# antonior92/ip-nonlinear-solver

Hardware: AMD Instinct MI355X
Metric: projected-CG iters/sec (fp64) at n=1e6,m=1e5 (higher is better)
Workload: dtype f64; 1 GPU; config3: sparse banded NLP subproblem, CSR Jacobian bandwidth 15: ONE call ipsolver.qp.projected_cg(H, c, Z, Y, b, trust_radius=1e300, tol=0, max_iter=steps), b a device vector (zeros; x0 = Y(-b) is computed: whether a device vector is zero is not known without reading it) -- priming included; finite trust radius that is never reached (the norm test of qp_subproblem.py:583 formed every iteration, ; n=1000000, m=100000, nnz_A=1500000, nnz_H=2999998, parallelism=single GPU

## Files before the change

include/ipx.h:

```cpp
#ifndef IPX_H
#define IPX_H

#include <stdint.h>

#ifdef __cplusplus
extern "C" {
#endif

#define IPX_OK 0
#define IPX_EINVAL (-1)
#define IPX_ELAUNCH (-2)
#define IPX_ENOTSPD (-3)
#define IPX_ENOMEM (-4)
#define IPX_EUNSUPPORTED (-5)
#define IPX_EILLCOND (-6)

#define IPX_WS_DOUBLES 65536
#define IPX_MAX_PARTIALS 2048

const char *ipx_version(void);
long long ipx_launch_count(void);
long long ipx_read_count(void);
const char *ipx_last_error(void);
int ipx_device_info(int *cu_count, int *lds_bytes, char *arch, int arch_len);
// ... 139 lines not shown
  const int32_t *A_rowptr, *A_colidx; const double *A_val; const int32_t *A_tiles; int64_t A_ntiles;
  const int32_t *At_rowptr, *At_colidx; const double *At_val; const int32_t *At_tiles; int64_t At_ntiles;
  const int32_t *H_rowptr, *H_colidx; const double *H_val; const int32_t *H_tiles; int64_t H_ntiles;
  const double *H_diag;
  void *banded;
  double *x, *p, *r, *Hp;
  double *w, *v, *t;
  const double *lb, *ub;
  double *state;
  double *part1, *part2, *part3, *part4;
  int64_t vec_grid;
  int64_t solver_kind;
  double *pb;
  int64_t H_hmax;
  int64_t H_tile_rows;
  double *r_next;
  const int32_t *A_own;
  int64_t A_span;
  double *fold_ws;
  const int32_t *At_vown;
  int64_t At_qv;
  int64_t A_tile_nnz;
  const uint16_t *At_ell_row;
  const double *At_ell_val;
  const void *H_col16;
  const int32_t *H_rowlen;
  const void *A_col16;
  int64_t no_radius;
  const void *A_off16;
  const int32_t *A_rowfirst;
  int64_t A_rl;
  const int32_t *P_win;
  int64_t P_nspan;
  int64_t P_navn;
  int64_t H_operator;
  int64_t resident;
  void *R_ll;
  int64_t R_hw;
  int64_t *R_seq;
  const double *LR_W;
  const double *LR_state;
  double *LR_part;
  int64_t LR_mem;
  int64_t LR_rows;
  double *xsums;
  int64_t fused_proj;
  const double *A_ell_val;
  const void *A_ell_off16;
  int32_t *r_where;
  int32_t xsums_carry;
  int32_t A_contig;
  double *rguard;
  int32_t radius_guard;
} ipx_cg_args;
#define IPX_CG_MODE_NO_RADIUS 1
#define IPX_CG_MODE_NO_ORTH 2
#define IPX_CG_MODE_CARRIED 4
#define IPX_CG_MODE_GUARD 8
#define IPX_CG_STOP_RADIUS_UNDECIDED 10
#define IPX_CG_STOP_GUARD_LOST 11
double ipx_rguard_start(double sumsq);
double ipx_rguard_step_x(double X, double Q, double alpha);
double ipx_rguard_step_q(double Q, double beta, double gg);
int ipx_cg_guard_resume(const ipx_cg_args *a, int32_t it_stop, void *stream);
int ipx_cg_prime_state_guard(double *state, const double *red, const int32_t *idx7, double tol_in,
                             double radius, double orth_tol, double norm_A, double cancellation,
                             double *rguard, void *stream);
int ipx_cg_resident_ok(const ipx_cg_args *a);
int64_t ipx_cg_resident_ll_words(int32_t nwg, int32_t hw);
void ipx_cg_resident_limits(int32_t *out8);
int32_t ipx_cg_resident_max_global(void);
int ipx_cg_state_size(void);
int ipx_cg_vec_grid(int64_t n);
int ipx_cg_hp(const ipx_cg_args *a, void *stream);
int ipx_cg_iterate(const ipx_cg_args *a, int32_t it_begin, int32_t it_end, void *stream);
int64_t ipx_cg_prime_ws_doubles(const ipx_cg_args *a, int32_t A_ntiles);
int ipx_cg_prime(const ipx_cg_args *a, const int32_t *A_tiles, int32_t A_ntiles, const double *c,
                 const double *b, double *red, double *ws, double tol_in, double radius,
                 double orth_tol, double norm_A, double cancellation, int32_t first_end,
                 int32_t steps, void *stream);
int ipx_cg_prime_state(double *state, const double *red, const int32_t *idx7, double tol_in,
                       double radius, double orth_tol, double norm_A, double cancellation,
                       void *stream);
int ipx_cg_iterate_timed(const ipx_cg_args *a, int32_t it_begin, int32_t it_end,
                         float *ms_out, void *stream);
int ipx_cg_step1(int64_t n, double *state, int32_t it, const double *p1, int32_t np1,
                 const double *x, const double *p, double *r, const double *Hp, const double *lb,
                 const double *ub, double *part2, int32_t grid, void *stream);
int ipx_cg_step2(int64_t n, double *state, int32_t it, int32_t mode, const double *p2,
                 int32_t np2, const double *p3, int32_t np3, const double *p4, int32_t np4,
                 double *x, double *p, const double *g, int32_t grid, void *stream);
typedef struct ipx_pcg_args {
  int64_t m, n;
  const int32_t *A_rowptr, *A_colidx; const double *A_val; const int32_t *A_tiles; int64_t A_ntiles;
  const int32_t *At_rowptr, *At_colidx; const double *At_val; const int32_t *At_tiles; int64_t At_ntiles;
  const double *dinv;
  double *v, *r, *p, *Sp;
  double *t;
  double *state;
  double *part1, *part2;
  int64_t grid;
  const double *binv; const int32_t *border; int64_t nblk;
  double *z, *part3;
  double *rsum; const int32_t *coarse_of, *goff; int64_t ncoarse;
  const double *X; int64_t ldx;
  double *y, *partc;
} ipx_pcg_args;
int ipx_pcg_state_size(void);
int ipx_pcg_iterate(const ipx_pcg_args *a, int32_t it_begin, int32_t it_end, void *stream);
int ipx_pcg_coarse_max(void);
int ipx_pcg_coarse_grid(int64_t ncoarse);
int ipx_pcg_precond_apply(const ipx_pcg_args *a, const double *r, double *z, double *rz,
                          void *stream);
int ipx_csr_aggregate_rows(int64_t ncoarse, const int32_t *A_rowptr, const int32_t *A_colidx,
                           const double *A_val, const int32_t *order, const int32_t *goff,
                           const int32_t *C_rowptr, const int32_t *C_colidx, double *C_val,
                           void *stream);
int ipx_aggregate_greedy(int64_t n, const int32_t *rowptr, const int32_t *colidx, int32_t cap,
                         int32_t *agg);
int ipx_blockjacobi_build(int64_t nblk, const int32_t *rowptr, const int32_t *colidx,
                          const double *val, const int32_t *order, double *binv, int *flag,
                          void *stream);
int ipx_blockjacobi_apply(int64_t m, int64_t nblk, const int32_t *order, const double *binv,
                          const double *r, double *z, double *ws, const double *state,
                          void *stream);
typedef struct ipx_shard2_ext {
  double *s1;
  double *pack;
  int64_t nseg;
  int64_t own_lo[4], own_hi[4];
  int64_t p1_lo[4], p1_hi[4];
  int64_t p3_lo[4], p3_hi[4];
  int64_t p2_lo, p2_hi;
  int64_t p4_lo, p4_hi;
  void *peer;
  int64_t seg_lo[4], seg_hi[4];
  int64_t send_left[4], send_right[4];
  int64_t fuse_comm;
  int64_t res_wg0, res_nwg, res_gwg0, res_gnwg;
} ipx_shard2_ext;
int ipx_cg_shard2_fusable(const ipx_cg_args *a, const ipx_shard2_ext *e);
int ipx_cg_shard2_segment(const ipx_cg_args *a, const ipx_shard2_ext *e, int32_t phase,
                          int32_t it, int32_t mode, void *stream);
int ipx_cg_shard2_iterate(const ipx_cg_args *a, const ipx_shard2_ext *e, int32_t it_begin,
                          int32_t it_end, void *stream);
int ipx_cg_shard2_resident_ok(const ipx_cg_args *a, const ipx_shard2_ext *e);
int ipx_cg_shard2_resident(const ipx_cg_args *a, const ipx_shard2_ext *e, int32_t it_begin,
                           int32_t it_end, void *stream);
int ipx_cg_save_pb(const ipx_cg_args *a, void *stream);

int ipx_peer_handle_bytes(void);
void *ipx_peer_create(int32_t rank, int32_t world, int64_t halo_cap);
int ipx_peer_export(void *peer, void *handle_out);
int ipx_peer_import(void *peer, int32_t rank, const void *handle_in);
int ipx_peer_ready(void *peer);
int64_t ipx_peer_halo_capacity(void *peer);
int ipx_peer_set_timeout(void *peer, double seconds);
int ipx_peer_sequence(void *peer, int64_t *out2);
int64_t ipx_peer_fused_launches(void *peer);
void ipx_peer_destroy(void *peer);
int ipx_peer_allreduce(void *peer, int32_t nq, const double *in, double *out, int *failed,
                       int32_t reps, void *stream);
int ipx_peer_allgather(void *peer, int32_t nq, const double *vals, double *out, int *failed,
                       void *stream);
int ipx_peer_exchange(void *peer, double *v, int32_t nseg, const int64_t *geom, int *failed,
                      void *stream);
// ... 224 lines not shown
```

ip-nonlinear-solver_amd/csrc/banded.hip:

```cpp
#include "ipx_common.h"
#include "pcr_window.h"
#include <vector>

namespace {

constexpr int KMAX = 8;
constexpr int MAX_LEVELS = 8;
constexpr int WIDE_MIN_ROWS = 2048;
constexpr int ITER_TOP_MIN_ROWS = 1024;
constexpr double ITER_ETA_MAX = 0.5;

struct Level {
  int m, k, c, P, q;
  int mR;
  double *band;
  double *Dinv;
  double *L;
  double *V, *W;
  double *rhs;
  double *sol;
};

struct Banded {
  int nlev;
// ... 1167 lines not shown
    }
    if (!partial) return;
  }
  double acc = 0.0;
  for (int r = threadIdx.x; r < T * q; r += blockDim.x) {
    const int64_t g = (int64_t)t0 * q + r;
    if (g < m) {
      const int li = q + r;
      double sum = sB[r] * sx[li];
#pragma unroll
      for (int d = 1; d <= K; ++d) {
        if (g - d >= 0) sum += sB[d * NB + r] * sx[li - d];
        if (g + d < m) sum += sB[d * NB + r + d] * sx[li + d];
      }
      const double res = sw0[r] - sum;
      acc += res * res;
    }
  }
  const double tot = ipx_block_reduce<IPX_SUM>(acc, red_lds);
  if (threadIdx.x == 0) partial[blockIdx.x] = tot;
  IPX_STAMP(7);
}


constexpr int PCR_RMAX = 4 * 66 + 2 * (1 << PCR_LMAX) + 8;
constexpr int PCR_NR = (PCR_RMAX + IPX_BLOCK - 1) / IPX_BLOCK;
constexpr int PCR_TB = 512;

__global__ void __launch_bounds__(IPX_BLOCK)
k_pcr_check(int m, int rows_wg, int nwin, const double *__restrict__ band, int *flags) {
  constexpr int PAD = PCR_PAD;
  constexpr int RS = PCR_RMAX + 2 * PAD;
  __shared__ double pa[2][RS], pr[2][RS];
  const int wg = ipx_xcd_item(blockIdx.x, nwin);
  if (wg < 0) return;
  const int tid = threadIdx.x;
  const PcrWindow win(wg, rows_wg, PCR_LMAX, m, tid);
  const int R = win.R;
  double a[PCR_NR], b[PCR_NR], b0[PCR_NR];
  bool own[PCR_NR];
#pragma unroll
  for (int k = 0; k < PCR_NR; ++k) {
    const int r = tid + k * IPX_BLOCK;
    win.row_load(band, r, a[k], b[k]);
    b0[k] = b[k];
    own[k] = win.own(r);
  }
  pcr_pad_identity<IPX_BLOCK, false>(R, tid, pa, pr);
  const double tiny = 1.3877787807814457e-17;
  for (int s = 0; s < PCR_LMAX; ++s) {
    const int h = 1 << s, cur = s & 1;
#pragma unroll
    for (int k = 0; k < PCR_NR; ++k) {
      const int r = tid + k * IPX_BLOCK;
      if (r < R) { pa[cur][PAD + r] = a[k]; pr[cur][PAD + r] = ipx_rcp_newton(b[k]); }
    }
    ipx_lds_barrier();
    int bits = 0;
#pragma unroll
    for (int k = 0; k < PCR_NR; ++k) {
      const int r = PAD + min(tid + k * IPX_BLOCK, R - 1);
      const double alo = pa[cur][r - h], rlo = pr[cur][r - h];
      const double ahi = pa[cur][r + h], rhi = pr[cur][r + h];
      double none = 0.0;
      pcr_eliminate<false>(a[k], b[k], none, alo, rlo, 0.0, ahi, rhi, 0.0);
      const double bn = b[k];
      if (own[k]) {
        const double aup = (-pa[cur][r + 2 * h] * rhi) * ahi;
        if (!(fmax(fabs(a[k]), fabs(aup)) <= tiny * bn)) bits |= 1;
        if (!(bn > 0.0)) bits |= 2;
        if (!(bn > IPX_PIVOT_RTOL * b0[k])) bits |= 4;
      }
    }
    const bool any0 = __ballot(bits & 1) != 0, any1 = __ballot(bits & 2) != 0;
    const bool any2 = __ballot(bits & 4) != 0;
    if ((tid & (IPX_WAVE - 1)) == 0) {
      if (any0) flags[s + 1] = 1;
      if (any1) flags[PCR_LMAX + 1 + s + 1] = 1;
      if (any2) flags[PCR_LMAX + 1] = 1;
    }
  }
}

template <int QV, int NR, bool ROWS, int TB, bool POST = false>
__global__ void __launch_bounds__(TB)
k_solve_pcr(int m, int rows_wg, int L, int nwin, const double *__restrict__ band,
            const double *__restrict__ w, double *__restrict__ x, double *__restrict__ partial,
            const double *__restrict__ guard, AtvJob atv, RowsJob rows = RowsJob{},
            PostJob post = PostJob{}) {
  constexpr int QA = QV > 0 ? QV : 1;
  constexpr int RS = PCR_RMAX + 2 * PCR_PAD;
  __shared__ double pa[2][RS], pr[2][RS], pd[2][RS];
  __shared__ double sx[PCR_RMAX];
  __shared__ double red_lds[TB / IPX_WAVE];
  constexpr int RWU = ROWS_PRODUCTS / TB;
  const int wg = ipx_xcd_item(blockIdx.x, nwin);
  if (wg < 0) return;
  IPX_STAMP(0);
  int av0 = 0, avn = 0;
  if (QV > 0) {
    av0 = atv.vown[wg];
    avn = atv.vown[wg + 1] - av0;
  }
  const double stop = guard ? *guard : 0.0;
  const int tid = threadIdx.x;
  const PcrWindow win(wg, rows_wg, L, m, tid);
  const int H = win.H, R = win.R;
  const int64_t g0 = win.row(0);
  extern __shared__ double rows_prod[];
  int rcol[ROWS ? RWU : 1];
  double rval[ROWS ? RWU : 1];
  if constexpr (ROWS) {
    const int64_t nnz = (int64_t)m << rows.logL;
    const int64_t e0 = g0 * (1 << rows.logL);
    const int P = R << rows.logL;
#pragma unroll
    for (int u = 0; u < RWU; ++u) {
      const int e = min(tid + u * TB, P - 1);
      const int64_t idx = min(max(e0 + e, (int64_t)0), nnz - 1);
      rcol[u] = rows.col[idx];
      rval[u] = rows.val[idx];
    }
  }
  double a[NR], b[NR], d[NR];
#pragma unroll
  for (int k = 0; k < NR; ++k) {
    const bool in = win.row_load(band, tid + k * TB, a[k], b[k]);
    if constexpr (!ROWS) {
      const double wv = w[win.clamped(tid + k * TB)];
      d[k] = in ? wv : 0.0;
    }
  }
  if constexpr (ROWS) {
    const int Lr = 1 << rows.logL, P = R << rows.logL;
    double xg[RWU];
#pragma unroll
    for (int u = 0; u < RWU; ++u) xg[u] = rows.x[rcol[u]];
#pragma unroll
    for (int u = 0; u < RWU; ++u) {
      const int e = tid + u * TB;
      if (e < P) rows_prod[(e >> rows.logL) * (Lr + 1) + (e & (Lr - 1))] = rval[u] * xg[u];
    }
    ipx_lds_barrier();
#pragma unroll
    for (int k = 0; k < NR; ++k) {
      const int r = tid + k * TB;
      const bool in = win.inside(r);
      double sum = 0.0;
      if (in) {
        const double *pr_ = rows_prod + r * (Lr + 1);
        for (int j = 0; j < Lr; ++j) sum += pr_[j];
      }
      d[k] = in ? 1.0 * sum : 0.0;
    }
  }
  constexpr int QP = (QA + 1) / 2;
  PcrPairTail<QP, TB> tail;
  v2d ar[QP];
  if (QV > 0)
    tail.load(atv.ell_row, atv.ell_val, atv.ell_n, av0, avn, tid, [&](int k, int64_t j) {
      ar[k] = *reinterpret_cast<const v2d *>(atv.r_in + j);
    });
  int pg0 = 0, pgn = 0, pe0 = 0, pen = 0;
  int py0[POST ? POST_PG + 1 : 1], py1[POST ? POST_PG + 1 : 1];
  double pw0[POST ? POST_PG + 1 : 1], pw1[POST ? POST_PG + 1 : 1];
  double pep[POST ? POST_PG : 1], peq[POST ? POST_PG : 1];
  double prc[POST ? POST_PG + 1 : 1], prp[POST ? POST_PG : 1], prq[POST ? POST_PG : 1];
  if constexpr (POST) {
    pg0 = post.own_g[wg]; pgn = post.own_g[wg + 1] - pg0;
    pe0 = post.own_e[wg]; pen = post.own_e[wg + 1] - pe0;
    const ipx_group_tab &T = post.T;
#pragma unroll
    for (int k = 0; k < POST_PG; ++k) {
      const int i = pg0 + min(tid + k * TB, max(pgn - 1, 0));
      const int gi = min(i, max(post.ng - 1, 0));
      const int c = T.c0 + gi;
      py0[k] = post.yrow[gi]; py1[k] = post.yrow[post.nitems + gi];
      pw0[k] = post.yval[gi]; pw1[k] = post.yval[post.nitems + gi];
      pep[k] = T.grp2[2 * gi]; peq[k] = T.grp2[2 * gi + 1];
      prc[k] = post.r[c]; prp[k] = post.r[c + T.dp]; prq[k] = post.r[c + T.dq];
    }
    {
      const int e = min(pe0 + min(tid, max(pen - 1, 0)), max(post.nitems - post.ng - 1, 0));
      const int i = post.ng + e;
      py0[POST_PG] = post.yrow[min(i, post.nitems - 1)];
      py1[POST_PG] = post.yrow[post.nitems + min(i, post.nitems - 1)];
      pw0[POST_PG] = post.yval[min(i, post.nitems - 1)];
      pw1[POST_PG] = post.yval[post.nitems + min(i, post.nitems - 1)];
      prc[POST_PG] = post.r[T.gen0 + e];
    }
  }
  if (stop != 0.0) return;
  IPX_STAMP(1);
  double a0[NR], b0[NR], w0[NR];
#pragma unroll
  for (int k = 0; k < NR; ++k) { a0[k] = a[k]; b0[k] = b[k]; w0[k] = d[k]; }
  IPX_STAMP(2);
  pcr_pad_identity<TB, true>(R, tid, pa, pr, pd);
  pcr_levels<NR, TB>(L, R, tid, a, b, d, pa, pr, pd);
  IPX_STAMP(3);
  pcr_solution_to_lds<NR, TB>(win, tid, d, b, sx, x);
  if (!partial && QV == 0 && !POST) return;
  ipx_lds_barrier();
  IPX_STAMP(6);
  if (QV > 0) {
    const double gacc = tail.apply(
        sx, H, atv.sign, tid, atv.g_out,
        [&](int k, int64_t, int half) { return half ? ar[k].y : ar[k].x; }, [](int, bool, bool) {});
    pcr_partial_pair<TB>(gacc, red_lds, atv.part3, wg, nwin, tid);
    if (!partial) return;
  }
  if constexpr (POST) {
    const ipx_group_tab &T = post.T;
    const int wlim = R - 1;
    double acc = 0.0;
#pragma unroll
    for (int k = 0; k < POST_PG; ++k) {
      if (tid + k * TB < pgn) {
        const int gi = pg0 + tid + k * TB;
        const int c = T.c0 + gi, cp = c + T.dp, cq = c + T.dq;
        const double u0 = sx[min(max((int)(py0[k] - g0), 0), wlim)];
        const double u1 = sx[min(max((int)(py1[k] - g0), 0), wlim)];
        double sum = 0.0;
        sum += pw0[k] * u0;
        sum += pw1[k] * u1;
        const double yj = 1.0 * sum;
        const double ap = copysign(1.0, pep[k]), sp = fabs(pep[k]);
        const double aq = copysign(1.0, peq[k]), sq = fabs(peq[k]);
        const double rc = prc[k], rp = prp[k], rq = prq[k];
        double i11, i12, i22, wgt;
        ipx_group_inverse(true, ap, sp, aq, sq, i11, i12, i22, wgt);
        const double wp = cp > c ? ap * rc + sp * rp : sp * rp + ap * rc;
        const double wq = cq > c ? aq * rc + sq * rq : sq * rq + aq * rc;
        const double ep = ap * yj, eq = aq * yj;
        const double tp = i11 * wp + i12 * wq;
        const double tq = i12 * wp + i22 * wq;
        const double vp = tp - (i11 * ep + i12 * eq);
        const double vq = tq - (i12 * ep + i22 * eq);
        double s3 = yj + ap * vp;
        s3 += aq * vq;
        double gc = -1.0 * s3;
        gc += 1.0 * rc;
        double gp = -1.0 * (sp * vp);
        gp += 1.0 * rp;
        double gq = -1.0 * (sq * vq);
        gq += 1.0 * rq;
        post.g[c] = gc; post.g[cp] = gp; post.g[cq] = gq;
        acc += gc * gc;
        acc += gp * gp;
        acc += gq * gq;
      }
    }
    if (tid < pen) {
      const int e = pe0 + tid;
      const double u0 = sx[min(max((int)(py0[POST_PG] - g0), 0), wlim)];
      const double u1 = sx[min(max((int)(py1[POST_PG] - g0), 0), wlim)];
      double sum = 0.0;
      sum += pw0[POST_PG] * u0;
      sum += pw1[POST_PG] * u1;
      double gc = -1.0 * (1.0 * sum);
      gc += 1.0 * prc[POST_PG];
      post.g[T.gen0 + e] = gc;
      acc += gc * gc;
    }
    const double gtot = ipx_block_reduce<IPX_SUM>(acc, red_lds);
    if (tid == 0) {
      post.part[wg] = gtot;
      post.part[post.count + wg] = 0.0;
      for (int k = wg + nwin; k < post.count; k += nwin) {
        post.part[k] = 0.0;
        post.part[post.count + k] = 0.0;
      }
    }
    if (!partial) return;
  }
  const double acc = pcr_own_residual<NR, TB>(win, tid, a0, b0, w0, pa[0], sx);
  const double tot = ipx_block_reduce<IPX_SUM>(acc, red_lds);
  if (tid == 0) partial[wg] = tot;
  IPX_STAMP(7);
}

template <int QV>
int launch_solve_pcr_q(const LevDev &lv, int L, const double *w, double *x, double *partial,
                       int *npartial, const double *guard, const AtvJob &atv, hipStream_t st) {
  const int rows_wg = DEC_CHUNKS * lv.q;
  const int grid = (lv.P + DEC_CHUNKS - 1) / DEC_CHUNKS;
  if (npartial) *npartial = grid;
  constexpr int NRL = (PCR_RMAX + PCR_TB - 1) / PCR_TB;
  if (rows_wg + 2 * (1 << L) <= PCR_TB)
    hipLaunchKernelGGL((k_solve_pcr<QV, 1, false, PCR_TB>), dim3(ipx_xcd_grid(grid)), dim3(PCR_TB),
                       0, st, lv.m, rows_wg, L, grid, lv.band, w, x, partial, guard, atv, RowsJob{});
  else
    hipLaunchKernelGGL((k_solve_pcr<QV, NRL, false, PCR_TB>), dim3(ipx_xcd_grid(grid)),
                       dim3(PCR_TB), 0, st, lv.m, rows_wg, L, grid, lv.band, w, x, partial, guard,
                       atv, RowsJob{});
  IPX_CHECK_LAUNCH();
  return IPX_OK;
}

int launch_solve_pcr_rows(const LevDev &lv, int L, const RowsJob &rows, double *x,
                          double *partial, int *npartial, const double *guard, hipStream_t st,
                          const PostJob *post = nullptr) {
  const int rows_wg = DEC_CHUNKS * lv.q;
  const int R = rows_wg + 2 * (1 << L);
  if (R > PCR_TB || ((int64_t)R << rows.logL) > (int64_t)ROWS_PRODUCTS)
    return IPX_EUNSUPPORTED;
  const int grid = (lv.P + DEC_CHUNKS - 1) / DEC_CHUNKS;
  if (npartial) *npartial = grid;
  const size_t lds = (size_t)R * ((1 << rows.logL) + 1) * sizeof(double);
  constexpr int dyn = (int)(LDS_LIMIT - 44 * 1024);
  if (post) {
    allow_dynamic_lds<k_solve_pcr<0, 1, true, PCR_TB, true>>(dyn);
    hipLaunchKernelGGL((k_solve_pcr<0, 1, true, PCR_TB, true>), dim3(ipx_xcd_grid(grid)),
                       dim3(PCR_TB), lds, st, lv.m, rows_wg, L, grid, lv.band, nullptr, x, partial,
                       guard, AtvJob{}, rows, *post);
  } else {
    allow_dynamic_lds<k_solve_pcr<0, 1, true, PCR_TB>>(dyn);
    hipLaunchKernelGGL((k_solve_pcr<0, 1, true, PCR_TB>), dim3(ipx_xcd_grid(grid)), dim3(PCR_TB),
                       lds, st, lv.m, rows_wg, L, grid, lv.band, nullptr, x, partial, guard,
                       AtvJob{}, rows);
  }
  IPX_CHECK_LAUNCH();
  return IPX_OK;
}

int pcr_tail_per_lane(int qv) { return (qv * (DOWN_T - IPX_WAVE) + 1 + PCR_TB - 1) / PCR_TB; }

int launch_solve_pcr(const LevDev &lv, int L, const double *w, double *x, double *partial,
                     int *npartial, const double *guard, hipStream_t st,
                     const AtvJob *atv = nullptr, int qv = 0) {
  const AtvJob none{};
  if (!atv || qv <= 0)
    return launch_solve_pcr_q<0>(lv, L, w, x, partial, npartial, guard, none, st);
  const int per = pcr_tail_per_lane(qv);
  if (per <= 2) return launch_solve_pcr_q<2>(lv, L, w, x, partial, npartial, guard, *atv, st);
  if (per <= 4) return launch_solve_pcr_q<4>(lv, L, w, x, partial, npartial, guard, *atv, st);
  if (per <= 6) return launch_solve_pcr_q<6>(lv, L, w, x, partial, npartial, guard, *atv, st);
  if (per <= 8) return launch_solve_pcr_q<8>(lv, L, w, x, partial, npartial, guard, *atv, st);
  return IPX_EINVAL;
}

template <int QV, int XN, bool PRIME = false, bool CONTIG = false>
__global__ void __launch_bounds__(PCR_TB)
k_step1_solve_tail(int m, int rows_wg, int L, int nwin, const double *__restrict__ band,
                   ipx_fused_proj_job J) {
  constexpr int TB = PCR_TB;
  constexpr int PAD = 1 << PCR_LMAX;
  constexpr int RS = PCR_RMAX + 2 * PAD;
  constexpr int QSP = IPX_FP_SPAN / TB;
  constexpr int RLA = IPX_FP_ROW;
  constexpr int FW = IPX_BLOCK, FU = 6;
  constexpr int QP = (QV + 1) / 2;
  __shared__ double pa[2][RS], pr[2][RS], pd[2][RS];
  __shared__ double sx[PCR_RMAX];
  __shared__ double span[IPX_FP_SPAN];
  __shared__ double red_lds[TB / IPX_WAVE];
  __shared__ double fold_lds[FW / IPX_WAVE];
  const int tid = threadIdx.x, wg = ipx_xcd_item(blockIdx.x, nwin);
  if (wg < 0) return;
  const int av0 = J.vown[wg], avn = J.vown[wg + 1] - av0;
  const int c_lo = J.win[2 * wg], nspan = J.win[2 * wg + 1] - c_lo;
  static_assert(!PRIME || XN == 1, "the priming's projection forms no radius test");
  double stop, rtg = 0.0, tol = 0.0;
  if constexpr (PRIME) {
    stop = J.guard ? *J.guard : 0.0;
  } else {
    stop = J.st[ST_STOP];
    rtg = J.st[J.parity ? ST_RTG1 : ST_RTG0];
    tol = J.st[ST_TOL];
  }
  double rgX = 0.0, rgQ = 0.0;
  if constexpr (XN == 3) {
    if (wg == 0 && tid == 0) { rgX = J.xs_comp[IPX_RG_X]; rgQ = J.xs_comp[IPX_RG_Q]; }
  }
  double ft[FU];
  if (!PRIME && tid < FW) {
#pragma unroll
    for (int u = 0; u < FU; ++u) {
      const int i = tid + u * FW;
      const double ld = J.p1[max(min(i, J.np1 - 1), 0)];
      ft[u] = i < J.np1 ? ld : 0.0;
    }
// ... 907 lines not shown
  }
  if (h->decoupled && w != x && h->pcr_L > 0 && h->lev[0].k == 1)
    return launch_solve_pcr(to_dev(h->lev[0], nullptr), h->pcr_L, w, x, partial, npartial, guard,
                            st);
  if (h->chunk_pending) {
    const int rc = ensure_chunks(h, st);
    if (rc != IPX_OK) return rc;
    return fast_solve(h, w, x, partial, npartial, guard, st);
  }
  if (h->decoupled && w != x)
    return solve_decoupled_k(to_dev(h->lev[0], nullptr), w, x, h->rinv, partial, npartial, guard,
                             st);
  if (h->iter_N > 0 && !h->decoupled) {
    if (w == x && partial) return IPX_EINVAL;
    return iter_solve(h, w, x, partial, npartial, guard, st);
  }
  if (h->wide) return IPX_EUNSUPPORTED;
  int rc = fast_down0(h, w, h->ybuf, guard, st);
  if (rc != IPX_OK) return rc;
  if (!decoupled_scalar(h)) {
    if (!h->upper_done) {
      rc = factor_upper(h, st);
      if (rc != IPX_OK) return rc;
    }
    rc = fast_middle(h, guard, st);
    if (rc != IPX_OK) return rc;
  }
  switch (h->lev[0].k) {
#define CO(kk) case kk: return launch_correct_oop<kk>(h, x, w, partial, npartial, guard, st)
    CO(1); CO(2); CO(3); CO(4); CO(5); CO(6); CO(7); CO(8);
#undef CO
  }
  return IPX_EINVAL;
}
}

int ipx_banded_resid_count(void *handle) {
  if (!handle) return 0;
  Banded *h = (Banded *)handle;
  const Level &l0 = h->lev[0];
  if (h->fast && h->nlev > 1 && h->decoupled)
    return (l0.P + DEC_CHUNKS - 1) / DEC_CHUNKS;
  if (h->fast && h->nlev > 1 && h->iter_N == 0) return (l0.m + IPX_BLOCK - 1) / IPX_BLOCK;
  const int grid = (l0.m + IPX_BLOCK - 1) / IPX_BLOCK;
  return grid > 256 ? 256 : grid;
}

extern "C" int ipx_banded_decoupled_geometry(void *handle, int32_t *out) {
  if (!handle || !out) return 0;
  Banded *h = (Banded *)handle;
  const Level &l0 = h->lev[0];
  if (!(h->fast && h->nlev > 1 && h->decoupled))
    return 0;
  out[0] = DEC_CHUNKS * l0.q;
  out[1] = (l0.P + DEC_CHUNKS - 1) / DEC_CHUNKS;
  return 1;
}

int ipx_banded_solve_resid_atv_launch(void *handle, const double *w, double *x, double *partial,
                                      int *npartial, const int32_t *At_rowptr,
                                      const int32_t *At_colidx, const double *At_val,
                                      const double *r_in, double *g_out, const int32_t *vown,
                                      int qv, double *part3, const double *guard,
                                      hipStream_t st, const uint16_t *ell_row,
                                      const double *ell_val, int64_t ell_n, double sign) {
  if (!handle || !w || !x || !partial || w == x || (sign != 1.0 && sign != -1.0)) return IPX_EINVAL;
  int32_t geo[2];
  if (!ipx_banded_decoupled_geometry(handle, geo)) return IPX_EINVAL;
  Banded *h = (Banded *)handle;
  const AtvJob job{At_rowptr, At_colidx, At_val, r_in, g_out, vown, part3, ell_row, ell_val, ell_n,
                   sign};
  if (h->pcr_L > 0 && ell_row && ell_val)
    return launch_solve_pcr(to_dev(h->lev[0], nullptr), h->pcr_L, w, x, partial, npartial, guard,
                            st, &job, qv);
  if (h->chunk_pending) {
    const int rc = ensure_chunks(h, st);
    if (rc != IPX_OK) return rc;
    if (!ipx_banded_decoupled_geometry(handle, geo)) return IPX_EINVAL;
  }
  return solve_decoupled_k(to_dev(h->lev[0], nullptr), w, x, h->rinv, partial, npartial, guard, st,
                           &job, qv);
}

int ipx_banded_fused_proj_ok(void *handle, int rl, int64_t nspan, int qv) {
  int32_t geo[2];
  if (!handle || !ipx_banded_decoupled_geometry(handle, geo)) return IPX_EUNSUPPORTED;
  Banded *h = (Banded *)handle;
  if (h->pcr_L <= 0 || h->lev[0].k != 1 || geo[0] + 2 * (1 << h->pcr_L) > PCR_TB)
    return IPX_EUNSUPPORTED;
  if (rl < 1 || rl > IPX_FP_ROW || nspan < 1 || nspan > IPX_FP_SPAN || qv < 1 ||
      pcr_tail_per_lane(qv) > 6)
    return IPX_EUNSUPPORTED;
  return IPX_OK;
}

int ipx_banded_fused_proj_launch(void *handle, const ipx_fused_proj_job &job, int *npartial,
                                 hipStream_t st) {
  if (job.prime ? (job.xn != 1 || (job.sign != 1.0 && job.sign != -1.0))
                : (!job.st || !job.p1 || !job.Hp || !job.where))
    return IPX_EINVAL;
  if (!job.r_in || !job.g_out || job.g_out == job.r_in ||
      !job.A_ell_val || !job.A_ell_off16 || !job.A_rowfirst || !job.win || !job.vown ||
      !job.ell_row || !job.ell_val || !job.v || !job.part3 || !job.part4 ||
      (job.n & 1) || (job.xn == 0 && (!job.x || !job.p || !job.part2)) ||
      (job.xn == 2 && (!job.xs_raw || !job.xs_comp || job.nraw < 1)) ||
      (job.xn == 3 && !job.xs_comp) || job.xn < 0 || job.xn > 3)
    return IPX_EINVAL;
  if (ipx_banded_fused_proj_ok(handle, job.rl, 1, job.qv) != IPX_OK) return IPX_EUNSUPPORTED;
  Banded *h = (Banded *)handle;
  const LevDev lv = to_dev(h->lev[0], nullptr);
  const int grid = (lv.P + DEC_CHUNKS - 1) / DEC_CHUNKS;
  if (job.xn == 2 && job.ncomp > grid) return IPX_EINVAL;
  if (npartial) *npartial = grid;
  const int per = pcr_tail_per_lane(job.qv);
  if (per <= 2) return launch_step1_solve_tail_q<2>(lv, h->pcr_L, job, grid, st);
  if (per <= 4) return launch_step1_solve_tail_q<4>(lv, h->pcr_L, job, grid, st);
  return launch_step1_solve_tail_q<6>(lv, h->pcr_L, job, grid, st);
}

int ipx_banded_pcr_view(void *handle, ipx_pcr_view *out) {
  if (!handle || !out) return 0;
  int32_t g2[2];
  if (!ipx_banded_decoupled_geometry(handle, g2)) return 0;
  Banded *h = (Banded *)handle;
  if (h->pcr_L <= 0) return 0;
  out->m = h->lev[0].m;
  out->rows_wg = g2[0];
  out->nwg = g2[1];
  out->L = h->pcr_L;
  out->band = h->lev[0].band;
  return 1;
}

int ipx_banded_solve_resid_launch(void *handle, const double *w, double *x, double *partial,
                                  int *npartial, const double *guard, hipStream_t st) {
  if (!handle || !w || !x || !partial || w == x) return IPX_EINVAL;
  Banded *h = (Banded *)handle;
  if (h->fast) return fast_solve(h, w, x, partial, npartial, guard, st);
  int rc = ipx_banded_solve_guarded(handle, w, x, guard, st);
  if (rc != IPX_OK) return rc;
  return ipx_banded_residual_launch(handle, w, x, partial, npartial, guard, st);
}

int ipx_banded_solve_rows_launch(void *handle, const int32_t *col, const double *val,
                                 const double *xin, int logL, double *x, double *partial,
                                 int *npartial, const double *guard, hipStream_t st,
                                 const ipx_post_job *pj) {
  if (!handle || !col || !val || !xin || !x || !partial || logL < 0 || logL > 4) return IPX_EINVAL;
  Banded *h = (Banded *)handle;
  if (!(h->fast && h->nlev > 1 && h->decoupled && h->pcr_L > 0)) return IPX_EUNSUPPORTED;
  const LevDev lv = to_dev(h->lev[0], nullptr);
  if (lv.k != 1) return IPX_EUNSUPPORTED;
  if (!pj)
    return launch_solve_pcr_rows(lv, h->pcr_L, RowsJob{col, val, xin, logL}, x, partial, npartial,
                                 guard, st);
  if (pj->rows_wg != DEC_CHUNKS * lv.q || pj->reach > 1 || (1 << h->pcr_L) < pj->reach)
    return IPX_EUNSUPPORTED;
  if ((lv.P + DEC_CHUNKS - 1) / DEC_CHUNKS > pj->count) return IPX_EUNSUPPORTED;
  PostJob post{pj->own_g, pj->own_e, pj->ng, pj->nitems, pj->T, pj->yrow, pj->yval, pj->r, pj->g,
               pj->part, pj->count};
  return launch_solve_pcr_rows(lv, h->pcr_L, RowsJob{col, val, xin, logL}, x, partial, npartial,
                               guard, st, &post);
}

int ipx_banded_solve_guarded(void *handle, const double *w, double *x, const double *guard,
                             hipStream_t st) {
// ... 85 lines not shown
```

ip-nonlinear-solver_amd/csrc/cg.hip:

```cpp
#include "ipx_common.h"
#include <algorithm>
#include <vector>


namespace {

IPX_STAMP_DECL(ipx_dbg_cg);
#define CG_STAMP(k) IPX_STAMP_TO(ipx_dbg_cg, k)

constexpr int VB = IPX_BLOCK;

constexpr int VU = 8;

typedef ipx_own_ranges OwnRanges;
struct ipx_no_peer {};
template <bool PEER> struct peer_arg { typedef ipx_no_peer type; };
template <> struct peer_arg<true> { typedef ipx_peer_job type; };
static OwnRanges own_all(int64_t n) {
  OwnRanges o;
  for (int k = 0; k < 4; ++k) { o.lo[k] = 0; o.hi[k] = 0; }
  o.hi[0] = n;
  return o;
}

// ... 770 lines not shown
  }
  int rpv[(IPX_SPMV_TILE_ROWS / IPX_BLOCK) + 1];
#pragma unroll
  for (int q = 0; q <= IPX_SPMV_TILE_ROWS / IPX_BLOCK; ++q)
    rpv[q] = rowptr[r0 + min(tid + q * IPX_BLOCK, nrows)] - s;
  CG_STAMP(11);
  ipx_lds_barrier();
  CG_STAMP(12);
#pragma unroll
  for (int u = 0; u < U; ++u) {
    const int jj = s + tid + u * IPX_BLOCK;
    if (jj < e) prod[jj - s] = v[u] * span[c[u]];
  }
#pragma unroll
  for (int q = 0; q <= IPX_SPMV_TILE_ROWS / IPX_BLOCK; ++q) {
    const int i = tid + q * IPX_BLOCK;
    if (i <= nrows) rp[i] = rpv[q];
  }
  ipx_lds_barrier();
  double yq[IPX_SPMV_TILE_ROWS / IPX_BLOCK];
#pragma unroll
  for (int q = 0; q < IPX_SPMV_TILE_ROWS / IPX_BLOCK; ++q) {
    const int i = tid + q * IPX_BLOCK;
    yq[q] = 0.0;
    if (i < nrows) {
      const int a = rp[i], b = rp[i + 1];
      double sum = 0.0;
      for (int k = a; k < b; ++k) sum += prod[k];
      yq[q] = 1.0 * sum;
    }
  }
  CG_STAMP(13);
  if (!NOXN2) {
    const double tot = ipx_block_reduce<IPX_SUM>(sx, lds);
    if (tid == 0) { part2[tile] = tot; part2[ntiles + tile] = 0.0; }
  }
#pragma unroll
  for (int q = 0; q < IPX_SPMV_TILE_ROWS / IPX_BLOCK; ++q) {
    const int i = tid + q * IPX_BLOCK;
    if (i < nrows) w[r0 + i] = yq[q];
  }
  CG_STAMP(14);
}

struct CompactJob {
  const double *in[3];
  double *out[3];
  int count[3], halves[3], G[3], first[4];
};
__global__ void __launch_bounds__(IPX_BLOCK)
k_compact_partials(CompactJob job, const double *__restrict__ guard) {
  __shared__ double lds[IPX_BLOCK / IPX_WAVE];
  if (guard && *guard != 0.0) return;
  int k = 0;
  while (k < 2 && (int)blockIdx.x >= job.first[k + 1]) ++k;
  const int b = blockIdx.x - job.first[k];
  const int half = b / job.G[k], chunk = b - half * job.G[k];
  const int lo = chunk * 1024, len = min(1024, job.count[k] - lo);
  const double v = ipx_sum_partials<IPX_SUM>(job.in[k] + (int64_t)half * job.count[k] + lo, len, lds);
  if (threadIdx.x == 0) job.out[k][half * job.G[k] + chunk] = v;
}

__global__ void __launch_bounds__(IPX_BLOCK)
k_cg_save_pb(const double *__restrict__ p, const int32_t *__restrict__ tiles, int ntiles,
             int hmax, double *__restrict__ pb, double *__restrict__ xs_tag) {
  const int idx = blockIdx.x * blockDim.x + threadIdx.x;
  if (idx == 0 && xs_tag) *xs_tag = 0.0;
  if (idx >= ntiles * 2 * hmax) return;
  const int t = idx / (2 * hmax), j = idx - t * 2 * hmax;
  const int r0 = tiles[t], r1 = tiles[t + 1];
  const double v = j < hmax ? p[r0 + j] : p[r1 - hmax + (j - hmax)];
  pb[idx] = v;
  pb[(int64_t)ntiles * 2 * hmax + idx] = v;
}

__global__ void __launch_bounds__(VB)
k_cg_settle_r(int64_t n, const int32_t *__restrict__ where, const double *__restrict__ src,
              double *__restrict__ dst) {
  if (*where == 0) return;
  for (int64_t i = (int64_t)blockIdx.x * VB + threadIdx.x; i < n; i += (int64_t)gridDim.x * VB)
    dst[i] = src[i];
}

__global__ void k_xsums_void(double *xs_tag) { *xs_tag = 0.0; }

__global__ void k_rguard_advance(const double *__restrict__ st, int parity, double *rg) {
  if (st[ST_STOP] != 0.0) return;
  const double gg = st[parity ? ST_RTG0 : ST_RTG1];
  rg[IPX_RG_Q] = ipx_rguard::step_q(rg[IPX_RG_Q], st[ST_BETA], gg);
  rg[IPX_RG_X] = rg[IPX_RG_T];
}

__global__ void __launch_bounds__(IPX_BLOCK)
k_rguard_sums(int64_t n, const double *__restrict__ x, const double *__restrict__ p,
              double *__restrict__ comp) {
  __shared__ double lds[3 * (IPX_BLOCK / IPX_WAVE)];
  const int64_t per = (n + XS_STRIDE - 1) / XS_STRIDE;
  const int64_t lo = min((int64_t)blockIdx.x * per, n), hi = min(lo + per, n);
  double acc[3] = {0.0, 0.0, 0.0}, out[3];
  for (int64_t i = lo + threadIdx.x; i < hi; i += IPX_BLOCK) {
    const double xv = x[i], pv = p[i];
    acc[0] += xv * xv;
    acc[1] += xv * pv;
    acc[2] += pv * pv;
  }
  ipx_block_sum_multi<3>(acc, lds, out);
  if (threadIdx.x == 0) {
#pragma unroll
    for (int q = 0; q < 3; ++q) comp[q * XS_STRIDE + blockIdx.x] = out[q];
  }
}

struct RangeJob {
  const double *ptr[4][4];
  int count[4][4];
  int npieces;
  int active;
};

__global__ void __launch_bounds__(256)
k_cg_range_pack(RangeJob job, double *__restrict__ out, const double *__restrict__ guard) {
  __shared__ double lds[4 * 4];
  if (guard && *guard != 0.0) return;
  double acc[4] = {0.0, 0.0, 0.0, 0.0};
  for (int pc = 0; pc < job.npieces; ++pc) {
    double red[4];
    ipx_sum_partials_multi<4>(job.ptr[pc], job.count[pc], lds, red);
#pragma unroll
    for (int q = 0; q < 4; ++q) acc[q] += red[q];
  }
  if (threadIdx.x < 4 && ((job.active >> threadIdx.x) & 1)) out[threadIdx.x] = acc[threadIdx.x];
}

struct HaloPlan {
  int nseg;
  int seg_lo[4], own_lo[4], own_hi[4], seg_hi[4], send_left[4], send_right[4];
};

__global__ void __launch_bounds__(256)
k_cg_pack_comm(RangeJob job, double *__restrict__ out, ipx_peer_view pv, uint32_t seq,
               HaloPlan hp, double *__restrict__ g, uint32_t hseq, double *__restrict__ st) {
  __shared__ double lds[4 * 4];
  __shared__ double vals[IPX_MAX_PEERS * 4];
  const int tid = threadIdx.x;
  if (st[ST_STOP] == 7.0) return;
  const long long deadline = (long long)wall_clock64() + pv.timeout_ticks;
  if (blockIdx.x == 0) {
    double acc[4] = {0.0, 0.0, 0.0, 0.0};
    for (int pc = 0; pc < job.npieces; ++pc) {
      double red[4];
      ipx_sum_partials_multi<4>(job.ptr[pc], job.count[pc], lds, red);
#pragma unroll
      for (int q = 0; q < 4; ++q) acc[q] += red[q];
    }
    const int slot = seq & (IPX_PEER_SLOTS - 1);
    if (tid < 4 * pv.world) {
      const int r = tid >> 2, q = tid & 3;
      if ((job.active >> q) & 1) {
        const double mine = q == 0 ? acc[0] : (q == 1 ? acc[1] : (q == 2 ? acc[2] : acc[3]));
        ipx_ll_store(pv.mbox[r] + ipx_peer_scal_word(slot, pv.rank, q), mine, seq);
      }
    }
    bool ok = true;
    if (tid < 4 * pv.world) {
      const int r = tid >> 2, q = tid & 3;
      double v = 0.0;
// ... 190 lines not shown
               : step2_hp_forms<PEER, false, 4, 5>(box, c16, xsum, guard);
}


template <bool PEER>
int launch_step1_box(const ipx_cg_args *a, int it, const double *p1, int np1, int np2,
                     const OwnRanges &own, typename peer_arg<PEER>::type pj, hipStream_t st) {
  const ipx_boxschur_args *b = (const ipx_boxschur_args *)a->banded;
  const ipx_group_tab T = ipx_boxschur_tab(b);
  hipLaunchKernelGGL(step1_box_kernel<PEER>(ipx_group_mode(T)), dim3(ipx_xcd_grid(np2)),
                     dim3(IPX_BLOCK), 0, st, a->state, it & 1, p1, np1, a->x, a->p, a->r, a->Hp,
                     a->lb, a->ub, a->part2, np2, (int)b->ng, (int)b->ngen, T, b->gen_cols,
                     (int)b->ny, b->up, own, step1_box_rounds(b), pj);
  IPX_CHECK_LAUNCH();
  return IPX_OK;
}

template <bool PEER>
int launch_step1_ar(const ipx_cg_args *a, const LoopPlan &P, int it, const double *p1, int np1,
                    bool no_xn2, bool carried, bool guard, typename peer_arg<PEER>::type pj,
                    hipStream_t st) {
  if (carried && (PEER || no_xn2 || !a->xsums)) return IPX_EINVAL;
  if (guard && (PEER || no_xn2 || carried || !a->rguard)) return IPX_EINVAL;
  if (a->A_tile_nnz != 0) return IPX_EINVAL;
  const int qs = (int)((a->A_span + IPX_BLOCK - 1) / IPX_BLOCK);
  const auto k = step1_ar_kernel<PEER>(qs, guard ? 3 : carried ? 2 : no_xn2 ? 1 : 0,
                                       a->A_col16 != nullptr);
  if (!k) return IPX_EINVAL;
  const int nraw = carried ? (int)a->H_ntiles : 0;
  hipLaunchKernelGGL(k, dim3(ipx_xcd_grid((int)a->A_ntiles)), dim3(IPX_BLOCK), 0, st, (int)a->n,
                     a->state, it & 1, p1, np1, a->x, a->p, a->r, a->r_next, a->Hp, a->A_rowptr,
                     a->A_colidx, a->A_val, a->A_tiles, (int)a->A_ntiles, a->A_own, a->w,
                     a->part2, (const uint16_t *)a->A_col16, pj, carried ? a->xsums : nullptr,
                     nraw, guard ? a->rguard : carried ? a->xsums + 3 * nraw + 1 : nullptr,
                     carried ? P.xs_ncomp : 0, it);
  IPX_CHECK_LAUNCH();
  return IPX_OK;
}

template <bool PEER>
int launch_step2_hp(const ipx_cg_args *a, int it, int mode, const double *p2, int np2,
                    const double *p3, int np3, const double *p4, int np4,
                    typename peer_arg<PEER>::type pj, const ipx_xsums_job &xs, hipStream_t st,
                    const double *g = nullptr) {
  const bool guard = (mode & 8) != 0;
  const bool xsum = !guard && xs.raw != nullptr && (xs.write != 0 || (mode & 4) != 0);
  if ((mode & 4) && (!xsum || !xs.in || PEER || a->lb)) return IPX_EINVAL;
  if (guard && (!xs.raw || !xs.in || xs.write || (mode & 4) || PEER || a->lb)) return IPX_EINVAL;
  const bool small = a->H_tile_rows > 0 && a->H_tile_rows + 2 * a->H_hmax <= 3 * IPX_BLOCK;
  const bool c16 = a->H_col16 != nullptr && a->H_rowlen != nullptr;
  const auto k = step2_hp_kernel<PEER>(a->H_diag != nullptr, small, a->lb != nullptr, c16, xsum,
                                       guard);
  if (!k) return IPX_EINVAL;
  const int64_t half = a->H_ntiles * 2 * a->H_hmax;
  const double *pb_in = a->pb + (it & 1) * half;
  double *pb_out = a->pb + ((it + 1) & 1) * half;
  double *g_halo = PEER ? a->r : nullptr;
  hipLaunchKernelGGL(k, dim3(ipx_xcd_grid((int)a->H_ntiles)), dim3(IPX_BLOCK), 0, st, (int)a->n,
                     a->state, it & 1, mode, p2, np2, p3, np3, p4, np4, a->x, a->p,
                     g ? g : (const double *)a->r, a->H_rowptr, a->H_colidx, a->H_val, a->H_tiles,
                     (int)a->H_ntiles, a->H_diag, a->Hp, a->part1, (int)a->H_hmax, pb_in, pb_out,
                     (const uint16_t *)a->H_col16, a->H_rowlen, pj, g_halo, xs);
  IPX_CHECK_LAUNCH();
  return IPX_OK;
}

double *xsums_tag(const ipx_cg_args *a) {
  return a->xsums ? a->xsums + 3 * a->H_ntiles : nullptr;
}

int launch_save_pb(const ipx_cg_args *a, hipStream_t st) {
  const int tot = (int)(a->H_ntiles * 2 * a->H_hmax);
  hipLaunchKernelGGL(k_cg_save_pb, dim3((tot + IPX_BLOCK - 1) / IPX_BLOCK), dim3(IPX_BLOCK), 0, st,
                     a->p, a->H_tiles, (int)a->H_ntiles, (int)a->H_hmax, a->pb, xsums_tag(a));
  IPX_CHECK_LAUNCH();
  return IPX_OK;
}

int launch_lowrank(const ipx_cg_args *a, bool has_base, const double *guard, hipStream_t st) {
  return ipx_lowrank_cg_launch(a->n, a->LR_rows, (int)a->LR_mem, a->LR_W, a->LR_state, a->LR_part,
                               a->p, a->Hp, a->H_diag, has_base ? 1 : 0, a->part1, guard, st);
}

int launch_hp(const ipx_cg_args *a, const LoopPlan &P, const double *guard, hipStream_t st) {
  int rc = IPX_OK;
  switch (P.hp) {
    case HP_OPERATOR:
      return IPX_OK;
    case HP_LOWRANK:
      return launch_lowrank(a, false, guard, st);
    case HP_DENSE: {
      int np = 0;
      rc = ipx_dense_gemv_launch((int)a->n, (int)a->n, a->H_val, a->n, a->p, 1.0, a->H_diag, 0.0,
                                 nullptr, a->Hp, a->part1, &np, guard, st);
      break;
    }
    case HP_CSR: {
      ipx_csr_view H{(int)a->n, (int)a->n, a->H_rowptr, a->H_colidx, a->H_val, a->H_tiles,
                     (int)a->H_ntiles};
      rc = ipx_spmv_launch(H, a->p, 1.0, a->H_diag, 0.0, nullptr, a->Hp, a->part1, guard, st);
      break;
    }
  }
  if (!rc && P.lowrank_tail) rc = launch_lowrank(a, true, guard, st);
  if (rc || P.hp != HP_CSR || !P.fused_hp) return rc;
  return launch_save_pb(a, st);
}

struct Compactor {
  const ipx_cg_args *a;
  CompactJob job;
  const double *guard;
  int n = 0, used = 0;
  Compactor(const ipx_cg_args *args, const double *g) : a(args), guard(g) { job.first[0] = 0; }
  bool add(const double *&ptr, int &count, int halves, int limit) {
    if (!a->fold_ws || count <= limit || n >= 3) return false;
    const int G = (count + 1023) / 1024;
    if (used + halves * G > IPX_FOLD_WS_DOUBLES) return false;
    job.in[n] = ptr; job.count[n] = count; job.halves[n] = halves; job.G[n] = G;
    job.out[n] = a->fold_ws + used;
    job.first[n + 1] = job.first[n] + halves * G;
    ptr = a->fold_ws + used;
    count = G;
    used += halves * G;
    ++n;
    return true;
  }
  int launch(hipStream_t st) {
    if (n == 0) return IPX_OK;
    for (int k = n; k < 3; ++k) job.first[k + 1] = job.first[n];
    hipLaunchKernelGGL(k_compact_partials, dim3(job.first[n]), dim3(IPX_BLOCK), 0, st, job, guard);
    IPX_CHECK_LAUNCH();
    n = 0;
    job.first[0] = 0;
    return IPX_OK;
  }
};


struct HalfArgs {
  int it;
  int mode;
  const double *guard;
  const OwnRanges *own = nullptr;
  const ipx_peer_job *peer = nullptr;
  Compactor *cmp = nullptr;
  ipx_xsums_job xs{nullptr, nullptr, it, 0};
  hipEvent_t *ev = nullptr;
  bool flip = false, first = true;
  const double *g = nullptr;
};
#define MARK(i) do { if (h.ev) (void)hipEventRecord(h.ev[i], st); } while (0)

int launch_projection_half(const ipx_cg_args *a, const LoopPlan &P, const HalfArgs &h,
                           const double *p1, int np1, int *np2, int *np3, int *np4,
                           hipStream_t st) {
  MARK(0);
  int rc;
  if (h.cmp) {
    h.cmp->add(p1, np1, 2, 2048);
    rc = h.cmp->launch(st);
    if (rc) return rc;
  }
  if (P.proj == PJ_STEP1_SOLVE_TAIL) {
    if (h.peer || h.own) return IPX_EINVAL;
    const bool carried = (h.mode & 4) != 0, guarded = (h.mode & 8) != 0;
    if (carried && ((h.mode & 1) || !a->xsums)) return IPX_EINVAL;
    if (guarded && ((h.mode & 5) || !a->rguard)) return IPX_EINVAL;
    const int nraw = carried ? (int)a->H_ntiles : 0;
    ipx_fused_proj_job J{};
    J.st = a->state; J.parity = h.it & 1; J.p1 = p1 + np1; J.np1 = np1;
    J.r_in = h.flip ? a->r_next : a->r; J.Hp = a->Hp; J.g_out = h.flip ? a->r : a->r_next;
    J.xn = guarded ? 3 : carried ? 2 : (h.mode & 1) ? 1 : 0;
    J.x = a->x; J.p = a->p; J.part2 = a->part2;
    J.xs_raw = carried ? a->xsums : nullptr; J.nraw = nraw;
    J.xs_comp = guarded ? a->rguard : carried ? a->xsums + 3 * nraw + 1 : nullptr;
    J.ncomp = carried ? P.xs_ncomp : 0; J.it = h.it;
    J.A_ell_val = a->A_ell_val; J.A_ell_off16 = (const uint16_t *)a->A_ell_off16;
    J.contig = a->A_contig != 0;
    J.A_rowfirst = a->A_rowfirst; J.rl = (int)a->A_rl; J.win = a->P_win; J.n = a->n;
    J.vown = a->At_vown; J.qv = (int)a->At_qv; J.ell_row = a->At_ell_row; J.ell_val = a->At_ell_val;
    J.v = a->v; J.part3 = a->part3; J.part4 = a->part4;
    J.where = a->r_where; J.first = h.first ? 1 : 0; J.dest = h.flip ? 0 : 1;
    MARK(1); MARK(2);
    int np = 0;
    rc = ipx_banded_fused_proj_launch(a->banded, J, &np, st);
    if (rc) return rc;
    *np2 = *np3 = *np4 = np;
// ... 57 lines not shown
        rc = ipx_banded_solve_resid_atv_launch(a->banded, a->w, a->v, a->part4, np4, a->At_rowptr,
                                               a->At_colidx, a->At_val, r_in, a->r, a->At_vown,
                                               (int)a->At_qv, a->part3, h.guard, st,
                                               a->At_ell_row, a->At_ell_val, a->n);
        if (rc) return rc;
        *np3 = *np4;
        MARK(3);
        MARK(4);
      } else {
        if (a->solver_kind == 1)
          rc = ipx_boxschur_solve((const ipx_boxschur_args *)a->banded, a->w, a->v, a->part4, np4,
                                  h.guard, st);
        else
          rc = ipx_banded_solve_resid_launch(a->banded, a->w, a->v, a->part4, np4, h.guard, st);
        if (rc) return rc;
        MARK(3);
        ipx_csr_view At{(int)a->n, (int)a->m, a->At_rowptr, a->At_colidx, a->At_val, a->At_tiles,
                        (int)a->At_ntiles};
        rc = ipx_spmv_launch(At, a->v, -1.0, nullptr, 1.0, r_in, a->r, a->part3, h.guard, st);
        if (rc) return rc;
        MARK(4);
      }
      MARK(5);
      break;
    }
    case PJ_STEP1_SOLVE_TAIL:
      return IPX_EINVAL;
    case PJ_DENSE: {
      const int n = (int)a->n, m = (int)a->m, M = ((m + 31) / 32) * 32;
      int np = 0;
      rc = ipx_dense_gemv_launch(m, n, a->A_val, n, a->r, 1.0, nullptr, 0.0, nullptr, a->w,
                                 nullptr, &np, h.guard, st);
      if (rc) return rc;
      rc = ipx_dense_gemv_launch(M, M, (const double *)a->banded, M, a->w, 1.0, nullptr, 0.0,
                                 nullptr, a->v, nullptr, &np, h.guard, st);
      if (rc) return rc;
      rc = ipx_dense_gemv_launch(n, m, a->At_val, m, a->v, -1.0, nullptr, 1.0, a->r, a->r,
                                 a->part3, np3, h.guard, st);
      if (rc) return rc;
      rc = ipx_dense_gemv_launch(m, n, a->A_val, n, a->r, 1.0, nullptr, 0.0, nullptr, a->t,
                                 a->part4, np4, h.guard, st);
      if (rc) return rc;
      break;
    }
  }
  return IPX_OK;
}

int launch_update_half(const ipx_cg_args *a, const LoopPlan &P, const HalfArgs &h,
                       const double *p2, int np2, const double *p3, int np3, const double *p4,
                       int np4, hipStream_t st) {
  int rc;
  if (h.cmp) {
    if (!(h.mode & 13)) h.cmp->add(p2, np2, 2, 1024);
    h.cmp->add(p3, np3, 2, 2048);
    if (!(h.mode & 2)) h.cmp->add(p4, np4, 1, 1024);
    rc = h.cmp->launch(st);
    if (rc) return rc;
  }
  const double *g = h.g ? h.g : a->r;
  if (P.step2 == S2_FUSED_HP) {
    MARK(6);
    rc = h.peer ? launch_step2_hp<true>(a, h.it, h.mode, p2, np2, p3, np3, p4, np4, *h.peer, h.xs,
                                        st)
                : launch_step2_hp<false>(a, h.it, h.mode, p2, np2, p3, np3, p4, np4,
                                         ipx_no_peer{}, h.xs, st, g);
    if (!rc && P.lowrank_tail) rc = launch_lowrank(a, true, h.guard, st);
  } else {
    if (h.peer) return IPX_EINVAL;
    hipLaunchKernelGGL(k_cg_step2, dim3(ipx_xcd_grid((int)a->vec_grid)), dim3(VB), 0, st, a->n,
                       a->state, h.it & 1, h.mode, p2, np2, p3, np3, p4, np4, a->x, a->p, g,
                       (int)a->vec_grid);
    IPX_CHECK_LAUNCH();
    MARK(6);
    rc = launch_hp(a, P, h.guard, st);
  }
  if (rc) return rc;
  MARK(7);
  return IPX_OK;
}
#undef MARK

int cg_iterate(const ipx_cg_args *a, const LoopPlan &P, int32_t it_begin, int32_t it_end,
               hipStream_t st, hipEvent_t *ev) {
  if (P.proj == PJ_DENSE) {
    if (ev) return IPX_EINVAL;
  } else if (!ev && it_end > it_begin && ipx_cg_resident_ok(a)) {
    int rc = ipx_cg_resident_launch(a, it_begin, it_end, P.np1, P.np2, P.np3, P.np4, st);
    if (rc || !P.fused_hp) return rc;
    return launch_save_pb(a, st);
  }
  const double *guard = a->state + ST_STOP;
  if (a->xsums && !P.xsums && it_end > it_begin) {
    hipLaunchKernelGGL(k_xsums_void, dim3(1), dim3(1), 0, st, xsums_tag(a));
    IPX_CHECK_LAUNCH();
  }
  for (int it = it_begin; it < it_end; ++it) {
    const bool carried = P.xsums && !P.guard && (it > it_begin || a->xsums_carry != 0);
    Compactor cmp(a, guard);
    HalfArgs h{it, (P.proj == PJ_NONE ? 2 : 0) | (P.no_xn2 ? 1 : 0) | (carried ? 4 : 0) |
                       (P.guard ? 8 : 0), guard};
    if (P.proj != PJ_DENSE) h.cmp = &cmp;
    h.xs = ipx_xsums_job{a->xsums,
                         P.guard ? a->rguard : carried ? a->xsums + 3 * a->H_ntiles + 1 : nullptr,
                         it, P.xsums && !P.guard ? 1 : 0};
    h.ev = ev;
    h.first = it == it_begin;
    h.flip = P.proj == PJ_STEP1_SOLVE_TAIL && ((it - it_begin) & 1) != 0;
    if (P.proj == PJ_STEP1_SOLVE_TAIL) h.g = h.flip ? a->r : a->r_next;
    int np2 = 0, np3 = 0, np4 = 0;
    int rc = launch_projection_half(a, P, h, a->part1, P.np1, &np2, &np3, &np4, st);
    if (rc) return rc;
    rc = launch_update_half(a, P, h, a->part2, np2, a->part3, np3, a->part4, np4, st);
    if (rc) return rc;
  }
  if (P.proj == PJ_STEP1_SOLVE_TAIL && it_end > it_begin) {
    hipLaunchKernelGGL(k_cg_settle_r, dim3(ipx_grid_for(a->n, VB * 4, 1024)), dim3(VB), 0, st, a->n,
                       a->r_where, (const double *)a->r_next, a->r);
    IPX_CHECK_LAUNCH();
  }
  return IPX_OK;
}
}

IPX_STAMP_EXPORT(ipx_debug_stamps_cg, ipx_dbg_cg)

extern "C" {

int ipx_cg_state_size(void) { return ST_SIZE; }
int ipx_cg_vec_grid(int64_t n) { return ipx_grid_for(n, VB * 2, 512); }

int ipx_cg_step1(int64_t n, double *state, int32_t it, const double *p1, int32_t np1,
                 const double *x, const double *p, double *r, const double *Hp, const double *lb,
                 const double *ub, double *part2, int32_t grid, void *stream) {
  if (n < 0 || !state || !p1 || !part2 || grid < 1) return IPX_EINVAL;
  hipLaunchKernelGGL(k_cg_step1, dim3(ipx_xcd_grid(grid)), dim3(VB), 0, (hipStream_t)stream, n,
                     state, it & 1, p1, np1, x, p, r, Hp, lb, ub, part2, grid, own_all(n));
  IPX_CHECK_LAUNCH();
  return IPX_OK;
}

int ipx_cg_step2(int64_t n, double *state, int32_t it, int32_t mode, const double *p2,
                 int32_t np2, const double *p3, int32_t np3, const double *p4, int32_t np4,
                 double *x, double *p, const double *g, int32_t grid, void *stream) {
  if (n < 0 || !state || grid < 1) return IPX_EINVAL;
  hipLaunchKernelGGL(k_cg_step2, dim3(ipx_xcd_grid(grid)), dim3(VB), 0, (hipStream_t)stream, n,
                     state, it & 1, mode, p2, np2, p3, np3, p4, np4, x, p, g, grid);
  IPX_CHECK_LAUNCH();
  return IPX_OK;
}

static OwnRanges own_of(const ipx_shard2_ext *e) {
  OwnRanges o;
  for (int k = 0; k < 4; ++k) {
    o.lo[k] = k < e->nseg ? e->own_lo[k] : 0;
    o.hi[k] = k < e->nseg ? e->own_hi[k] : 0;
  }
  return o;
}

static int launch_pack(const ipx_cg_args *a, const ipx_shard2_ext *e, const RangeJob &job,
                       double *out, bool with_halo, hipStream_t st) {
  ipx_peer *peer = (ipx_peer *)e->peer;
  if (!peer) {
    hipLaunchKernelGGL(k_cg_range_pack, dim3(1), dim3(256), 0, st, job, out,
                       (const double *)nullptr);
    IPX_CHECK_LAUNCH();
    return IPX_OK;
  }
  if (peer->view.world > IPX_MAX_PEERS || !ipx_peer_ready(peer)) return IPX_EINVAL;
  HaloPlan hp;
  hp.nseg = 0;
  int64_t moved = 0;
  if (with_halo && peer->view.world > 1) {
    hp.nseg = (int)e->nseg;
    int64_t inl = 0, inr = 0, outl = 0, outr = 0;
    for (int k = 0; k < hp.nseg; ++k) {
      hp.seg_lo[k] = (int)e->seg_lo[k]; hp.seg_hi[k] = (int)e->seg_hi[k];
      hp.own_lo[k] = (int)e->own_lo[k]; hp.own_hi[k] = (int)e->own_hi[k];
      hp.send_left[k] = (int)e->send_left[k]; hp.send_right[k] = (int)e->send_right[k];
      if (hp.seg_lo[k] > hp.own_lo[k] || hp.own_hi[k] > hp.seg_hi[k] || hp.send_left[k] < 0 ||
          hp.send_right[k] < 0 || hp.send_left[k] + hp.send_right[k] > 2 * (hp.own_hi[k] - hp.own_lo[k]))
        return IPX_EINVAL;
      inl += hp.own_lo[k] - hp.seg_lo[k]; inr += hp.seg_hi[k] - hp.own_hi[k];
      outl += hp.send_left[k]; outr += hp.send_right[k];
    }
    if (inl > peer->view.cap || inr > peer->view.cap || outl > peer->view.cap || outr > peer->view.cap)
      return IPX_EINVAL;
    moved = inl + inr + outl + outr;
    if (++peer->hseq == 0) ++peer->hseq;
  }
  if (++peer->seq == 0) ++peer->seq;
  const int halo_wg = hp.nseg ? (int)std::min<int64_t>(16, std::max<int64_t>(1, (moved + 511) / 512)) : 0;
  hipLaunchKernelGGL(k_cg_pack_comm, dim3(1 + halo_wg), dim3(256), 0, st, job, out, peer->view,
                     peer->seq, hp, a->r, peer->hseq, a->state);
  IPX_CHECK_LAUNCH();
  return IPX_OK;
// ... 192 lines not shown
    const double nx2 = q[1 + 3 * pj], nz2 = q[2 + 3 * pj], naz2 = q[3 + 3 * pj];
    const double nz = sqrt(nz2), naz = sqrt(naz2);
    const double orth = (nz == 0.0 || norm_A == 0.0) ? 0.0 : naz / (norm_A * nz);
    const bool stepped = taken && taken[pj] != 0.0;
    if (orth > orth_tol || (!stepped && nz2 < canc2 * nx2)) bad = true;
    if (!stepped && nx2 > 0.0) margin = fmin(margin, nz2 / nx2);
  }
  const double rt_g = q[5];
  const double tr_distance = radius - sqrt(q[0]);
  if (!(tr_distance >= 1e-25)) bad = true;
  double tol = tol_in;
  if (tol_in != tol_in) tol = fmax(fmin(0.01 * sqrt(rt_g), 0.1 * rt_g), 1e-25);
  for (int k = 0; k < ST_SIZE; ++k) st[k] = 0.0;
  st[ST_RTG0] = rt_g;
  st[ST_TOL] = tol;
  st[ST_RADIUS] = radius;
  st[ST_ORTH_RHS] = orth_tol * norm_A;
  st[ST_MARGIN] = margin;
  st[ST_PRIME_STEPS] = taken ? taken[0] + taken[1] : 0.0;
  st[ST_STOP] = bad ? 9.0 : 0.0;
  if (rguard) {
    rguard[IPX_RG_X] = ipx_rguard::start(q[0]);
    rguard[IPX_RG_Q] = ipx_rguard::start(rt_g);
    rguard[IPX_RG_T] = 0.0;
  }
}

__global__ void k_cg_prime_state(double *st, const double *__restrict__ red, ipx_prime_idx ix,
                                 double tol_in, double radius, double orth_tol, double norm_A,
                                 double canc2, double *rguard) {
  if (threadIdx.x != 0 || blockIdx.x != 0) return;
  prime_state_body(st, red, ix, tol_in, radius, orth_tol, norm_A, canc2, nullptr, rguard);
}

struct PrimeFolds {
  const double *part[6];
  int count[6], slot[6], n;
  int single[6];
};
#define PR_SKIP 14
#define PR_TAKEN 16
struct PrimeStep {
  const double *cz, *ct;
  int ncz, nct, base, pj;
  int pairs;
};
__device__ void prime_fold4(const double *pz, int npz, const double *pt, int npt, int pairs,
                            double *lds, double (&out)[4]) {
  const double *parts[4] = {pz, pairs ? pz + npz : pz, pt, pairs ? pt + npt : pt};
  const int counts[4] = {npz, pairs ? npz : 0, npt, pairs ? npt : 0};
  ipx_sum_partials_multi<4>(parts, counts, lds, out);
}
__device__ void prime_fold_step(double *red, const PrimeStep &c, double *lds) {
  if (red[PR_SKIP + c.pj] != 0.0) return;
  double out[4];
  prime_fold4(c.cz, c.ncz, c.ct, c.nct, c.pairs, lds, out);
  if (threadIdx.x == 0) {
    red[c.base] = out[0]; red[c.base + 1] = out[1];
    red[c.base + 2] = out[2]; red[c.base + 3] = out[3];
    red[PR_TAKEN + c.pj] = 1.0;
  }
  __syncthreads();
}
__global__ void __launch_bounds__(IPX_BLOCK)
k_prime_decide(double *red, const double *pz, int npz, const double *pt, int npt, int pairs,
               int base, int xslot, int pj, double orth_tol, double norm_A, double canc2,
               const double *__restrict__ norm_A2_dev, PrimeStep prev, int have_prev) {
  __shared__ double lds[4 * (IPX_BLOCK / IPX_WAVE)];
  if (have_prev) prime_fold_step(red, prev, lds);
  if (norm_A2_dev) norm_A = sqrt(*norm_A2_dev);
  double out[4];
  prime_fold4(pz, npz, pt, npt, pairs, lds, out);
  if (threadIdx.x != 0) return;
  red[base] = out[0]; red[base + 1] = out[1];
  red[base + 2] = out[2]; red[base + 3] = out[3];
  const double nx2 = red[xslot], nz2 = out[0], naz2 = out[2];
  const double nz = sqrt(nz2), naz = sqrt(naz2);
  const double orth = (nz == 0.0 || norm_A == 0.0) ? 0.0 : naz / (norm_A * nz);
  const bool need = orth > orth_tol || nz2 < canc2 * nx2;
  red[PR_SKIP + pj] = need ? 0.0 : 1.0;
  red[PR_TAKEN + pj] = 0.0;
}

__global__ void __launch_bounds__(IPX_BLOCK)
k_cg_prime_state_folds(double *st, double *red, PrimeFolds f, ipx_prime_idx ix, double tol_in,
                       double radius, double orth_tol, double norm_A, double canc2,
                       const double *__restrict__ radius_dev,
                       const double *__restrict__ norm_A2_dev, PrimeStep last, int have_last,
                       double *rguard) {
  if (radius_dev) radius = *radius_dev;
  if (norm_A2_dev) norm_A = sqrt(*norm_A2_dev);
  __shared__ double lds[12 * (IPX_BLOCK / IPX_WAVE)];
  const double *parts[12];
  int counts[12];
#pragma unroll
  for (int j = 0; j < 6; ++j) {
    const bool on = j < f.n, two = on && !f.single[j];
    parts[2 * j] = on ? f.part[j] : f.part[0];
    parts[2 * j + 1] = two ? f.part[j] + f.count[j] : f.part[0];
    counts[2 * j] = on ? f.count[j] : 0;
    counts[2 * j + 1] = two ? f.count[j] : 0;
  }
  double out[12];
  if (f.n > 0) {
    ipx_sum_partials_multi<12>(parts, counts, lds, out);
    if (threadIdx.x == 0) {
#pragma unroll
      for (int j = 0; j < 6; ++j)
        if (j < f.n) { red[f.slot[j]] = out[2 * j]; red[f.slot[j] + 1] = out[2 * j + 1]; }
    }
    __syncthreads();
  }
  if (have_last) prime_fold_step(red, last, lds);
  if (threadIdx.x == 0)
    prime_state_body(st, red, ix, tol_in, radius, orth_tol, norm_A, canc2,
                     have_last ? red + PR_TAKEN : nullptr, rguard);
}

int ipx_cg_prime_state_guard(double *state, const double *red, const int32_t *idx7,
                             double tol_in, double radius, double orth_tol, double norm_A,
                             double cancellation, double *rguard, void *stream) {
  if (!state || !red || !idx7) return IPX_EINVAL;
  ipx_prime_idx ix;
  for (int k = 0; k < 7; ++k) ix.i[k] = idx7[k];
  hipLaunchKernelGGL(k_cg_prime_state, dim3(1), dim3(64), 0, (hipStream_t)stream, state, red, ix,
                     tol_in, radius, orth_tol, norm_A, cancellation * cancellation, rguard);
  IPX_CHECK_LAUNCH();
  return IPX_OK;
}

int ipx_cg_prime_state(double *state, const double *red, const int32_t *idx7, double tol_in,
                       double radius, double orth_tol, double norm_A, double cancellation,
                       void *stream) {
  return ipx_cg_prime_state_guard(state, red, idx7, tol_in, radius, orth_tol, norm_A, cancellation,
                                  nullptr, stream);
}

static int prime_solve(const ipx_cg_args *a, const double *w, double *v, void *stream) {
  if (a->solver_kind == 1)
    return ipx_boxschur_solve((const ipx_boxschur_args *)a->banded, w, v, nullptr, nullptr, nullptr,
                              stream);
  return ipx_banded_solve(a->banded, w, v, stream);
}
struct PrimeRed {
  double *red, *ws;
  int64_t off;
  PrimeFolds f;
  int spmv(const ipx_csr_view &M, const double *x, double alpha, const double *diag, double beta,
           const double *yin, double *yout, int slot, hipStream_t st) {
    double *part = ws + off;
    off += 2 * (int64_t)M.ntiles;
    f.part[f.n] = part; f.count[f.n] = M.ntiles; f.slot[f.n] = slot; f.single[f.n] = 0; ++f.n;
    return ipx_spmv_launch(M, x, alpha, diag, beta, yin, yout, part, nullptr, st);
  }
  void single(const double *part, int count, int slot) {
    f.part[f.n] = part; f.count[f.n] = count; f.slot[f.n] = slot; f.single[f.n] = 1; ++f.n;
  }
};

static int prime_project(const ipx_cg_args *a, const ipx_csr_view &A, const ipx_csr_view &At,
                         const double *x, double *z, PrimeRed &R, int base, bool have_xnorm,
                         double sign, hipStream_t st) {
  int rc = have_xnorm ? IPX_OK : ipx_norms(a->n, x, R.red + base + 4, R.ws + R.off, st);
  if (rc) return rc;
  rc = ipx_spmv_launch(A, x, 1.0, nullptr, 0.0, nullptr, a->w, nullptr, nullptr, st);
  if (rc) return rc;
  rc = prime_solve(a, a->w, a->v, st);
  if (rc) return rc;
  rc = R.spmv(At, a->v, -sign, nullptr, sign, x, z, base, st);
  if (rc) return rc;
  return R.spmv(A, z, 1.0, nullptr, 0.0, nullptr, a->t, base + 2, st);
}
// ... 24 lines not shown
                             int base, bool have_xnorm, double sign, hipStream_t st) {
  if (P.proj != PJ_SOLVE_TAIL && P.proj != PJ_STEP1_SOLVE_TAIL)
    return prime_project(a, A, At, x, z, R, base, have_xnorm, sign, st);
  int rc = have_xnorm ? IPX_OK : ipx_norms(a->n, x, R.red + base + 4, R.ws + R.off, st);
  if (rc) return rc;
  const int cap = (int)((a->m + 255) / 256) + 8;
  double *pz = R.ws + R.off, *pt = pz + 2 * cap;
  R.off += 3 * (int64_t)cap;
  int np = 0;
  rc = prime_project_tail(a, P, A, x, z, pz, pt, &np, sign, nullptr, st);
  if (rc) return rc;
  R.single(pz, np, base);
  R.single(pt, np, base + 2);
  return IPX_OK;
}

static int prime_project_stepped(const ipx_cg_args *a, const LoopPlan &P,
                                 const ipx_csr_view &A, const ipx_csr_view &At, const double *x, double *z, PrimeRed &R,
                                 int base, int xslot, int pj, bool have_xnorm, double sign,
                                 double orth_tol, double norm_A, const double *norm_A2_dev,
                                 double canc2, const PrimeStep *prev, PrimeStep *step,
                                 hipStream_t st) {
  const int n0 = R.f.n;
  int rc;
  const double *skip = R.red + PR_SKIP + pj;
  if (P.proj == PJ_SOLVE_TAIL || P.proj == PJ_STEP1_SOLVE_TAIL) {
    if (!have_xnorm) {
      rc = ipx_norms(a->n, x, R.red + base + 4, R.ws + R.off, st);
      if (rc) return rc;
    }
    const int cap = (int)((a->m + 255) / 256) + 8;
    double *pz = R.ws + R.off, *pt = pz + 2 * cap, *cz = pt + cap, *ct = cz + 2 * cap;
    R.off += 6 * (int64_t)cap;
    int np = 0, npc = 0;
    rc = prime_project_tail(a, P, A, x, z, pz, pt, &np, sign, nullptr, st);
    if (rc) return rc;
    hipLaunchKernelGGL(k_prime_decide, dim3(1), dim3(IPX_BLOCK), 0, st, R.red, pz, np, pt, np, 0,
                       base, xslot, pj, orth_tol, norm_A, canc2, norm_A2_dev,
                       prev ? *prev : PrimeStep{}, prev ? 1 : 0);
    IPX_CHECK_LAUNCH();
    rc = prime_project_tail(a, P, A, z, z, cz, ct, &npc, 1.0, skip, st);
    if (rc) return rc;
    *step = PrimeStep{cz, ct, npc, npc, base, pj, 0};
    return IPX_OK;
  }
  rc = prime_project(a, A, At, x, z, R, base, have_xnorm, sign, st);
  if (rc) return rc;
  const double *pz = R.f.part[n0], *pt = R.f.part[n0 + 1];
  const int npz = R.f.count[n0], npt = R.f.count[n0 + 1];
  R.f.n = n0;
  hipLaunchKernelGGL(k_prime_decide, dim3(1), dim3(IPX_BLOCK), 0, st, R.red, pz, npz, pt, npt, 1,
                     base, xslot, pj, orth_tol, norm_A, canc2, norm_A2_dev,
                     prev ? *prev : PrimeStep{}, prev ? 1 : 0);
  IPX_CHECK_LAUNCH();
  if (a->solver_kind == 1)
    rc = ipx_boxschur_solve((const ipx_boxschur_args *)a->banded, a->t, a->v, nullptr, nullptr, skip,
                            st);
  else
    rc = ipx_banded_solve_guarded(a->banded, a->t, a->v, skip, st);
  if (rc) return rc;
  double *cz = R.ws + R.off;
  R.off += 2 * (int64_t)At.ntiles;
  double *ct = R.ws + R.off;
  R.off += 2 * (int64_t)A.ntiles;
  rc = ipx_spmv_launch(At, a->v, -1.0, nullptr, 1.0, z, z, cz, skip, st);
  if (rc) return rc;
  rc = ipx_spmv_launch(A, z, 1.0, nullptr, 0.0, nullptr, a->t, ct, skip, st);
  if (rc) return rc;
  *step = PrimeStep{cz, ct, At.ntiles, A.ntiles, base, pj, 1};
  return IPX_OK;
}

int64_t ipx_cg_prime_ws_doubles(const ipx_cg_args *a, int32_t A_ntiles) {
  if (!a) return -1;
  return 2 * (5 * a->At_ntiles + 4 * (int64_t)A_ntiles + a->H_ntiles) + 4096;
}

int ipx_cg_prime(const ipx_cg_args *a, const int32_t *A_tiles, int32_t A_ntiles, const double *c,
                 const double *b, double *red, double *ws, double tol_in, double radius,
                 double orth_tol, double norm_A, double cancellation, int32_t first_end,
                 int32_t steps, void *stream) {
  return ipx_cg_prime_dev(a, A_tiles, A_ntiles, c, b, red, ws, tol_in, radius, nullptr, orth_tol,
                          norm_A, nullptr, cancellation, first_end, steps, nullptr, 0, 0,
                          (hipStream_t)stream);
}

}

int ipx_cg_prime_dev(const ipx_cg_args *a, const int32_t *A_tiles, int32_t A_ntiles,
                     const double *c, const double *b, double *red, double *ws, double tol_in,
                     double radius, const double *radius_dev, double orth_tol, double norm_A,
                     const double *norm_A2_dev, double cancellation, int32_t first_end,
                     int steps, const double *c_part, int32_t c_npart, int x_is_zero,
                     hipStream_t stream) {
  if (!a || !c || !red || !ws || !A_tiles || a->solver_kind > 1 || a->m <= 0 || a->H_operator ||
      !a->H_rowptr || !a->t || first_end < 0 || a->LR_W)
    return IPX_EINVAL;
  hipStream_t st = (hipStream_t)stream;
  const LoopPlan P = plan_of(a);
  const ipx_csr_view A{(int)a->m, (int)a->n, a->A_rowptr, a->A_colidx, a->A_val, A_tiles, A_ntiles};
  const ipx_csr_view At{(int)a->n, (int)a->m, a->At_rowptr, a->At_colidx, a->At_val, a->At_tiles,
                        (int)a->At_ntiles};
  const ipx_csr_view Hm{(int)a->n, (int)a->n, a->H_rowptr, a->H_colidx, a->H_val, a->H_tiles,
                        (int)a->H_ntiles};
  if (ipx_cg_prime_ws_doubles(a, A_ntiles) > IPX_WS_DOUBLES) return IPX_EUNSUPPORTED;
  PrimeRed R{red, ws, 0, PrimeFolds{}};
  int rc;
  const double *t = c;
  if (b) {
    rc = prime_solve(a, b, a->v, stream);
    if (rc) return rc;
    rc = R.spmv(At, a->v, -1.0, nullptr, 0.0, nullptr, a->x, 12, st);
    if (rc) return rc;
    rc = R.spmv(Hm, a->x, 1.0, a->H_diag, 1.0, c, a->Hp, 4, st);
    if (rc) return rc;
    t = a->Hp;
  } else if (!x_is_zero &&
             hipMemsetAsync(a->x, 0, (size_t)a->n * sizeof(double), st) != hipSuccess) {
    return IPX_ELAUNCH;
  }
  const double canc2 = cancellation * cancellation;
  PrimeStep s1{}, s2{};
  if (b || !steps) {
    const bool c_known = !b && c_part && c_npart > 0;
    if (c_known) {
      PrimeFolds &f = R.f;
      f.part[f.n] = c_part; f.count[f.n] = c_npart; f.slot[f.n] = 4; f.single[f.n] = 0; ++f.n;
    }
    rc = prime_project_any(a, P, A, At, t, a->r, R, 0, b != nullptr || c_known, 1.0, st);
    if (rc) return rc;
    rc = prime_project_any(a, P, A, At, a->r, a->p, R, 6, true, -1.0, st);
    if (rc) return rc;
  } else {
    rc = prime_project_stepped(a, P, A, At, t, a->r, R, 0, 4, 0, false, 1.0, orth_tol, norm_A,
                               norm_A2_dev, canc2, nullptr, &s1, st);
    if (rc) return rc;
    rc = prime_project_stepped(a, P, A, At, a->r, a->p, R, 6, 0, 1, true, -1.0, orth_tol, norm_A,
                               norm_A2_dev, canc2, &s1, &s2, st);
    if (rc) return rc;
  }
  const int32_t idx_b[7] = {12, 4, 0, 2, 0, 6, 8}, idx_0[7] = {-1, 4, 0, 2, 0, 6, 8};
  ipx_prime_idx ix;
  for (int k = 0; k < 7; ++k) ix.i[k] = (b ? idx_b : idx_0)[k];
  hipLaunchKernelGGL(k_cg_prime_state_folds, dim3(1), dim3(IPX_BLOCK), 0, st, a->state, red, R.f,
                     ix, tol_in, radius, orth_tol, norm_A, canc2, radius_dev, norm_A2_dev, s2,
                     (b || !steps) ? 0 : 1, a->radius_guard != 0 ? a->rguard : nullptr);
  IPX_CHECK_LAUNCH();
  rc = launch_hp(a, P, nullptr, st);
  if (rc || first_end == 0) return rc;
  return cg_iterate(a, P, 0, first_end, st, nullptr);
}

extern "C" {

int ipx_cg_hp(const ipx_cg_args *a, void *stream) {
  if (!a) return IPX_EINVAL;
  return launch_hp(a, plan_of(a), nullptr, (hipStream_t)stream);
}

int ipx_cg_step2_hp(const ipx_cg_args *a, int32_t it, int32_t mode, void *stream) {
  if (!a || (mode & ~3)) return IPX_EINVAL;
  LoopPlan P = plan_of(a);
  if (!P.fused_hp) return IPX_EINVAL;
  P.step2 = S2_FUSED_HP;
  Compactor cmp(a, nullptr);
  HalfArgs h{it, mode, a->state + ST_STOP};
  h.cmp = &cmp;
  return launch_update_half(a, P, h, a->part2, P.np2, a->part3, P.np3, a->part4, P.np4,
                            (hipStream_t)stream);
}

int ipx_cg_resume(const ipx_cg_args *a, int32_t it, int32_t mode, void *stream) {
  if (!a) return IPX_EINVAL;
  LoopPlan P = plan_of(a);
  P.step2 = S2_VECTOR;
  const HalfArgs h{it, mode, a->state + ST_STOP};
  if (P.guard && !(mode & 1)) return IPX_EINVAL;
  int rc = launch_update_half(a, P, h, a->part2, P.np2, a->part3, P.np3, a->part4, P.np4,
                              (hipStream_t)stream);
  if (rc || !P.guard) return rc;
  hipLaunchKernelGGL(k_rguard_advance, dim3(1), dim3(1), 0, (hipStream_t)stream,
                     (const double *)a->state, it & 1, a->rguard);
  IPX_CHECK_LAUNCH();
  return IPX_OK;
}

int ipx_cg_guard_resume(const ipx_cg_args *a, int32_t it_stop, void *stream) {
  if (!a || !a->xsums || !a->rguard) return IPX_EINVAL;
  LoopPlan P = plan_of(a);
  if (!P.xsums || P.step2 != S2_FUSED_HP) return IPX_EINVAL;
  hipStream_t st = (hipStream_t)stream;
  double *comp = a->xsums + 3 * a->H_ntiles + 1;
  hipLaunchKernelGGL(k_rguard_sums, dim3(XS_STRIDE), dim3(IPX_BLOCK), 0, st, a->n,
                     (const double *)a->x, (const double *)a->p, comp);
  IPX_CHECK_LAUNCH();
  const double *guard = a->state + ST_STOP;
  Compactor cmp(a, guard);
  HalfArgs h{it_stop, 4, guard};
  h.cmp = &cmp;
  h.xs = ipx_xsums_job{a->xsums, comp, it_stop, 1};
  int rc = launch_update_half(a, P, h, a->part2, P.np2, a->part3, P.np3, a->part4, P.np4, st);
  if (rc) return rc;
  if (hipMemsetAsync(comp, 0, (size_t)3 * XS_STRIDE * sizeof(double), st) != hipSuccess)
    return IPX_ELAUNCH;
  return IPX_OK;
}

double ipx_rguard_start(double sumsq) { return ipx_rguard::start(sumsq); }
double ipx_rguard_step_x(double X, double Q, double alpha) {
  return ipx_rguard::step_x(X, Q, alpha);
}
double ipx_rguard_step_q(double Q, double beta, double gg) {
  return ipx_rguard::step_q(Q, beta, gg);
}

int ipx_cg_iterate(const ipx_cg_args *a, int32_t it_begin, int32_t it_end, void *stream) {
  if (!a || it_end < it_begin) return IPX_EINVAL;
  return cg_iterate(a, plan_of(a), it_begin, it_end, (hipStream_t)stream, nullptr);
}

#define IPX_CG_NCLASS 7
int ipx_cg_iterate_timed(const ipx_cg_args *a, int32_t it_begin, int32_t it_end, float *ms_out,
                         void *stream) {
  if (!a || it_end < it_begin || !ms_out) return IPX_EINVAL;
  hipStream_t st = (hipStream_t)stream;
  const LoopPlan P = plan_of(a);
  const int per_it = IPX_CG_NCLASS + 1;
  const int nit = it_end - it_begin;
  std::vector<hipEvent_t> ev((size_t)nit * per_it);
  for (auto &e : ev)
    if (hipEventCreate(&e) != hipSuccess) return IPX_ELAUNCH;
  int rc = IPX_OK;
  for (int i = 0; i < nit && rc == IPX_OK; ++i)
// ... 17 lines not shown
```

ip-nonlinear-solver_amd/csrc/ipx_common.h:

```cpp
#pragma once
#include <hip/hip_runtime.h>
#include <stdint.h>
#include "../../include/ipx.h"

#define IPX_BLOCK 256
#define IPX_WAVE 64
#define IPX_PIVOT_RTOL 1.1368683772161603e-13
#define IPX_VEC_GRID_CAP 1024

void ipx_note_error(hipError_t e, const char *file, int line);
int ipx_read_begin(unsigned int **pinned_out, unsigned int *tag_out);
int ipx_read_wait(unsigned int *pinned, unsigned int tag, int k, double *host_out, hipStream_t st);
int ipx_read_ints(const int *dev, int k, int *host_out, hipStream_t st);

int ipx_lowrank_cg_launch(int64_t n, int64_t rows, int mem, const double *W, const double *state,
                          double *part, const double *p, double *Hp, const double *diag,
                          int has_base, double *part1, const double *guard, hipStream_t st);

extern long long g_ipx_launches;

#define IPX_CHECK_LAUNCH()                                   \
  do {                                                       \
    ++g_ipx_launches;                                        \
    hipError_t e_ = hipGetLastError();                       \
    if (e_ != hipSuccess) {                                  \
      ipx_note_error(e_, __FILE__, __LINE__);                \
      return IPX_ELAUNCH;                                    \
    }                                                        \
  } while (0)

static inline int ipx_grid_for(int64_t n, int per_block, int cap = IPX_VEC_GRID_CAP) {
  int64_t g = (n + per_block - 1) / per_block;
  if (g < 1) g = 1;
  if (g > cap) g = cap;
  return (int)g;
}

static inline int ipx_xcd_grid(int nitems) { return 8 * ((nitems + 7) / 8); }
constexpr int IPX_NUM_CUS = 256;
static inline int ipx_balanced_rounds(int64_t items, int rmin, int rmax) {
  int best = rmin;
  int64_t cost = INT64_MAX;
  for (int R = rmin; R <= rmax; ++R) {
    const int64_t nb = (items + (int64_t)IPX_BLOCK * R - 1) / ((int64_t)IPX_BLOCK * R);
    const int64_t per_cu = (nb + IPX_NUM_CUS - 1) / IPX_NUM_CUS;
    const int64_t c = R * (per_cu < 2 ? 2 : per_cu);
    if (c < cost) { cost = c; best = R; }
  }
  return best;
}
__device__ __forceinline__ int ipx_xcd_item(int block, int nitems) {
  const int per = (nitems + 7) >> 3;
  const int t = (block & 7) * per + (block >> 3);
  return ((block >> 3) < per && t < nitems) ? t : -1;
}

template <int CTRL>
__device__ __forceinline__ double ipx_dpp(double v) {
  int lo = __double2loint(v), hi = __double2hiint(v);
  lo = __builtin_amdgcn_update_dpp(0, lo, CTRL, 0xf, 0xf, false);
  hi = __builtin_amdgcn_update_dpp(0, hi, CTRL, 0xf, 0xf, false);
  return __hiloint2double(hi, lo);
}
__device__ __forceinline__ double ipx_readlane(double v, int lane) {
  const int lo = __builtin_amdgcn_readlane(__double2loint(v), lane);
  const int hi = __builtin_amdgcn_readlane(__double2hiint(v), lane);
  return __hiloint2double(hi, lo);
}
#define IPX_WAVE_REDUCE(v, COMB)                                                  \
  do {                                                                            \
    v = COMB(v, ipx_dpp<0xB1>(v));                       \
    v = COMB(v, ipx_dpp<0x4E>(v));                       \
    v = COMB(v, ipx_dpp<0x141>(v));                      \
    v = COMB(v, ipx_dpp<0x140>(v));                      \
    const double r0 = ipx_readlane(v, 0), r1 = ipx_readlane(v, 16);               \
    const double r2 = ipx_readlane(v, 32), r3 = ipx_readlane(v, 48);              \
    v = COMB(COMB(r0, r1), COMB(r2, r3));                                         \
  } while (0)
#define IPX_ADD(a, b) ((a) + (b))
__device__ __forceinline__ double ipx_wave_sum(double v) {
  IPX_WAVE_REDUCE(v, IPX_ADD);
  return v;
}
__device__ __forceinline__ double ipx_wave_max(double v) {
  IPX_WAVE_REDUCE(v, fmax);
  return v;
}
__device__ __forceinline__ double ipx_wave_min(double v) {
  IPX_WAVE_REDUCE(v, fmin);
  return v;
}

__device__ __forceinline__ double ipx_rcp_newton(double b) {
  double r = __builtin_amdgcn_rcp(b);
// ... 336 lines not shown
                                                 double &sp, double &aq, double &sq) {
  if constexpr (UNIT) {
    const double ep = T.grp2[2 * g], eq = T.grp2[2 * g + 1];
    ap = copysign(1.0, ep); sp = fabs(ep);
    aq = copysign(1.0, eq); sq = fabs(eq);
  } else {
    ap = T.grp[4 * g]; sp = T.grp[4 * g + 1]; aq = T.grp[4 * g + 2]; sq = T.grp[4 * g + 3];
  }
}

__device__ __forceinline__ bool ipx_group_inverse(bool has_q, double ap, double sp, double aq,
                                                  double sq, double &i11, double &i12,
                                                  double &i22, double &wgt) {
  const double b11 = ap * ap + sp * sp;
  if (!has_q) {
    i11 = 1.0 / b11; i12 = 0.0; i22 = 0.0;
    wgt = sp * sp / b11;
    return b11 > 0.0;
  }
  const double b22 = aq * aq + sq * sq, b12 = ap * aq;
  const double det = ap * ap * (sq * sq) + sp * sp * (aq * aq) + sp * sp * (sq * sq);
  i11 = b22 / det; i12 = -b12 / det; i22 = b11 / det;
  wgt = (sp * sp) * (sq * sq) / det;
  return det > 0.0 && b11 > 0.0;
}

__device__ __forceinline__ void ipx_group_w(const ipx_group_tab &T, int g, const double *__restrict__ r,
                                        int &c, int &cp, int &cq, double &ap, double &sp,
                                        double &aq, double &sq, double &rc, double &rp, double &rq,
                                        double &wp, double &wq) {
  c = T.gcol[3 * g]; cp = T.gcol[3 * g + 1]; cq = T.gcol[3 * g + 2];
  ap = T.grp[4 * g]; sp = T.grp[4 * g + 1]; aq = T.grp[4 * g + 2]; sq = T.grp[4 * g + 3];
  rc = r[c];
  rp = cp >= 0 ? r[cp] : 0.0;
  rq = cq >= 0 ? r[cq] : 0.0;
  wp = cp < 0 ? ap * rc : (cp > c ? ap * rc + sp * rp : sp * rp + ap * rc);
  wq = cq < 0 ? aq * rc : (cq > c ? aq * rc + sq * rq : sq * rq + aq * rc);
}

#endif

#ifdef IPX_PHASE_TIMING
#define IPX_STAMP_DECL(name) __device__ unsigned long long name[16]
#define IPX_STAMP_TO(name, k) \
  do { if (blockIdx.x == 0 && threadIdx.x == 0) name[k] = wall_clock64(); } while (0)
#define IPX_STAMP_EXPORT(fn, name)                                                         \
  extern "C" int fn(unsigned long long *out) {                                             \
    return hipMemcpyFromSymbol(out, HIP_SYMBOL(name), 16 * sizeof(unsigned long long)) ==  \
                   hipSuccess ? 0 : -1;                                                    \
  }
#else
#define IPX_STAMP_DECL(name)
#define IPX_STAMP_TO(name, k) do { } while (0)
#define IPX_STAMP_EXPORT(fn, name)
#endif

enum {
  ST_RTG0 = 0, ST_RTG1 = 1,
  ST_TOL = 2, ST_RADIUS = 3, ST_ALPHA = 4, ST_STOP = 5, ST_NITER = 6, ST_BETA = 7,
  ST_PTHP = 8, ST_ORTH_RHS = 9,
  ST_XNORM2 = 10, ST_VIOL = 11, ST_ORTH = 12, ST_IT_DONE = 13,
  ST_MARGIN = 14,
  ST_PRIME_STEPS = 15,
  ST_SIZE = 16
};

struct ipx_prime_idx { int i[7]; };

struct ipx_pcr_view {
  int m, rows_wg, nwg, L;
  const double *band;
};
int ipx_banded_pcr_view(void *handle, ipx_pcr_view *out);
int ipx_cg_resident_launch(const ipx_cg_args *a, int32_t it_begin, int32_t it_end, int np1, int np2,
                           int np3, int np4, hipStream_t st);
int ipx_cg_shard2_resident_launch(const ipx_cg_args *a, const ipx_shard2_ext *e, int32_t it_begin,
                                  int32_t it_end, int np1, hipStream_t st);

int ipx_cg_prime_dev(const ipx_cg_args *a, const int32_t *A_tiles, int32_t A_ntiles,
                     const double *c, const double *b, double *red, double *ws, double tol_in,
                     double radius, const double *radius_dev, double orth_tol, double norm_A,
                     const double *norm_A2_dev, double cancellation, int32_t first_end,
                     int steps, const double *c_part, int32_t c_npart, int x_is_zero,
                     hipStream_t stream);

struct ipx_csr_view {
  int nrows, ncols;
  const int32_t *rowptr, *colidx;
  const double *val;
  const int32_t *tiles;
  int ntiles;
};
int ipx_spmv_launch(const ipx_csr_view &A, const double *x, double alpha, const double *diag,
                    double beta, const double *yin, double *yout, double *partial,
                    const double *guard, hipStream_t st, const double *xrow_override = nullptr);
int ipx_banded_solve_guarded(void *handle, const double *w, double *x, const double *guard,
                             hipStream_t st);
#ifdef __HIPCC__
struct ipx_post_job {
  const int32_t *own_g, *own_e;
  int ng, nitems;
  ipx_group_tab T;
  const int32_t *yrow;
  const double *yval;
  const double *r;
  double *g;
  double *part;
  int count, rows_wg, reach;
};
int ipx_banded_solve_rows_launch(void *handle, const int32_t *col, const double *val,
                                 const double *xin, int logL, double *x, double *partial,
                                 int *npartial, const double *guard, hipStream_t st,
                                 const ipx_post_job *post = nullptr);
#endif
int ipx_boxschur_project_from(const ipx_boxschur_args *a, const double *r, double *g,
                              double *part_g, int32_t *npart_g, double *part_res,
                              int32_t *npart_res, const double *guard, int have_up,
                              hipStream_t stream, const ipx_own_ranges *own = nullptr);
int ipx_dense_gemv_launch(int m, int n, const double *A, int64_t lda, const double *x,
                          double alpha, const double *diag, double beta, const double *yin,
                          double *yout, double *partial, int *npartial, const double *guard,
                          hipStream_t st);
int ipx_banded_resid_count(void *handle);
int ipx_banded_solve_resid_atv_launch(void *handle, const double *w, double *x, double *partial,
                                      int *npartial, const int32_t *At_rowptr,
                                      const int32_t *At_colidx, const double *At_val,
                                      const double *r_in, double *g_out, const int32_t *vown,
                                      int qv, double *part3, const double *guard,
                                      hipStream_t st, const uint16_t *ell_row = nullptr,
                                      const double *ell_val = nullptr, int64_t ell_n = 0,
                                      double sign = 1.0);
int ipx_banded_solve_resid_launch(void *handle, const double *w, double *x, double *partial,
                                  int *npartial, const double *guard, hipStream_t st);
constexpr int IPX_XS_SLICE = 64;
constexpr int IPX_XS_STRIDE = IPX_BLOCK;
constexpr int IPX_RG_X = 0, IPX_RG_Q = 1, IPX_RG_T = 2;
struct ipx_rguard {
  static constexpr double INFL = 1.0 + 0x1p-20;
  static __host__ __device__ inline double start(double sumsq) { return sqrt(sumsq) * INFL; }
  static __host__ __device__ inline double step_x(double X, double Q, double alpha) {
    return (X + fabs(alpha) * Q) * INFL;
  }
  static __host__ __device__ inline double step_q(double Q, double beta, double gg) {
    return (beta * Q + sqrt(gg)) * INFL;
  }
};
constexpr int IPX_FP_SPAN = 4096;
constexpr int IPX_FP_ROW = 16;
struct ipx_fused_proj_job {
  double *st;
  int parity;
  const double *p1; int np1;
  const double *r_in, *Hp;
  double *g_out;
  int xn;
  const double *x, *p;
  double *part2;
  const double *xs_raw; int nraw; double *xs_comp; int ncomp; int it;
  const double *A_ell_val; const uint16_t *A_ell_off16; const int32_t *A_rowfirst; int rl;
  int contig;
  const int32_t *win;
  int64_t n;
  const int32_t *vown; int qv;
  const uint16_t *ell_row; const double *ell_val;
  double *v, *part3, *part4;
  int32_t *where; int first, dest;
  int prime; double sign; const double *guard;
};
int ipx_banded_fused_proj_ok(void *handle, int rl, int64_t nspan, int qv);
int ipx_banded_fused_proj_launch(void *handle, const ipx_fused_proj_job &job, int *npartial,
                                 hipStream_t st);
int ipx_banded_residual_launch(void *handle, const double *w, const double *v, double *partial,
                               int *npartial, const double *guard, hipStream_t st);
```

ip-nonlinear-solver_amd/csrc/misc.hip:

```cpp
#include "ipx_common.h"
#include <string.h>
#include <stdio.h>
#include <atomic>
#include <chrono>

constexpr int IPX_READ_MAX = 512;
extern "C" int ipx_read_doubles(const double *dev, int k, double *host_out, void *stream);

typedef unsigned int ipx_u4 __attribute__((ext_vector_type(4)));
__global__ void __launch_bounds__(IPX_READ_MAX)
k_publish(const double *__restrict__ src, int k, ipx_u4 *dst, unsigned int tag) {
  if ((int)threadIdx.x >= k) return;
  const unsigned long long bits = (unsigned long long)__double_as_longlong(src[threadIdx.x]);
  ipx_u4 w;
  w.x = (unsigned)(bits & 0xffffffffull); w.y = tag;
  w.z = (unsigned)(bits >> 32);           w.w = tag;
  ipx_u4 *d = dst + threadIdx.x;
  asm volatile("global_store_dwordx4 %0, %1, off sc0 sc1" ::"v"(d), "v"(w) : "memory");
}

static thread_local char g_last_error[256] = "";
static std::atomic<long long> g_ipx_reads{0};

void ipx_note_error(hipError_t e, const char *file, int line) {
  snprintf(g_last_error, sizeof(g_last_error), "%s (%s:%d)", hipGetErrorString(e), file, line);
}

int ipx_read_begin(unsigned int **pinned_out, unsigned int *tag_out) {
  static thread_local unsigned int *pinned = nullptr;
  static thread_local unsigned int seq = 0;
  if (!pinned) {
    if (hipHostMalloc((void **)&pinned, IPX_READ_MAX * 16, hipHostMallocMapped | hipHostMallocCoherent) != hipSuccess) {
      pinned = nullptr;
      return IPX_ENOMEM;
    }
    memset(pinned, 0, IPX_READ_MAX * 16);
  }
  if (++seq == 0) ++seq;
  *pinned_out = pinned;
  *tag_out = seq;
  return IPX_OK;
}

int ipx_read_wait(unsigned int *pinned, unsigned int seq, int k, double *host_out, hipStream_t st) {
  volatile unsigned int *w = pinned;
  g_ipx_reads.fetch_add(1, std::memory_order_relaxed);
  const auto t0 = std::chrono::steady_clock::now();
  unsigned spins = 0;
  int done = 0;
  while (true) {
    while (done < k && w[4 * done + 1] == seq && w[4 * done + 3] == seq) ++done;
    if (done == k) break;
    __builtin_ia32_pause();
    if ((++spins & 0xfffu) == 0 &&
        std::chrono::steady_clock::now() - t0 > std::chrono::seconds(2)) {
      hipError_t e = hipStreamSynchronize(st);
      if (e != hipSuccess) { ipx_note_error(e, __FILE__, __LINE__); return IPX_ELAUNCH; }
      for (done = 0; done < k && w[4 * done + 1] == seq && w[4 * done + 3] == seq; ++done) {}
      if (done != k) return IPX_ELAUNCH;
      break;
    }
  }
  std::atomic_thread_fence(std::memory_order_acquire);
  for (int i = 0; i < k; ++i) {
    const unsigned long long bits = (unsigned long long)w[4 * i] | ((unsigned long long)w[4 * i + 2] << 32);
    memcpy(host_out + i, &bits, sizeof(double));
  }
  return IPX_OK;
}

struct FoldDescs { ipx_fold_desc d[IPX_FOLD_MAX]; };
__global__ void __launch_bounds__(IPX_BLOCK)
k_publish_folded(FoldDescs descs, int nd, ipx_u4 *dst, unsigned int tag) {
  __shared__ double lds[IPX_BLOCK / IPX_WAVE];
  for (int q = 0; q < nd; ++q) {
    const double *part = descs.d[q].part;
    const int count = descs.d[q].count, op = descs.d[q].op;
    double r;
    if (op == IPX_MAX) r = ipx_sum_partials<IPX_MAX>(part, count, lds);
    else if (op == IPX_MIN) r = ipx_sum_partials<IPX_MIN>(part, count, lds);
    else r = ipx_sum_partials<IPX_SUM>(part, count, lds);
    if (threadIdx.x == 0) {
      const unsigned long long bits = (unsigned long long)__double_as_longlong(r);
      ipx_u4 w;
      w.x = (unsigned)(bits & 0xffffffffull); w.y = tag;
      w.z = (unsigned)(bits >> 32);           w.w = tag;
      ipx_u4 *d = dst + q;
      asm volatile("global_store_dwordx4 %0, %1, off sc0 sc1" ::"v"(d), "v"(w) : "memory");
    }
    __syncthreads();
  }
}

struct FoldWeights { double w[IPX_FOLD_MAX]; };
__global__ void __launch_bounds__(IPX_BLOCK)
k_fold_combine(FoldDescs descs, FoldWeights wts, int nd, double *__restrict__ out) {
  __shared__ double lds[IPX_BLOCK / IPX_WAVE];
  double acc = 0.0;
  for (int q = 0; q < nd; ++q) {
    const double *part = descs.d[q].part;
    const int count = descs.d[q].count, op = descs.d[q].op;
    double r;
    if (op == IPX_MAX) r = ipx_sum_partials<IPX_MAX>(part, count, lds);
    else if (op == IPX_MIN) r = ipx_sum_partials<IPX_MIN>(part, count, lds);
    else r = ipx_sum_partials<IPX_SUM>(part, count, lds);
    const double term = wts.w[q] * r;
    acc = q == 0 ? term : acc + term;
    __syncthreads();
  }
  if (threadIdx.x == 0) out[0] = acc;
}

long long g_ipx_launches = 0;

extern "C" {

const char *ipx_version(void) { return "ipx 0.1 (gfx950)"; }

long long ipx_launch_count(void) { return g_ipx_launches; }

long long ipx_read_count(void) { return g_ipx_reads.load(); }

// ... 84 lines not shown
```

ip-nonlinear-solver_amd/ipsolver/_hip.py:

```python
import ctypes
import os

_HERE = os.path.dirname(os.path.abspath(__file__))
LIB_PATH = os.path.join(os.path.dirname(_HERE), "lib", "libipx.so")

WS_DOUBLES = 65536
VEC_GRID_CAP = 1024
SPMV_TILE_NNZ = 2048

_c = ctypes
_P, _I64, _I32, _F64 = _c.c_void_p, _c.c_int64, _c.c_int32, _c.c_double

_SIGNATURES = {
    "ipx_device_info": [_c.POINTER(_c.c_int), _c.POINTER(_c.c_int), _c.c_char_p, _c.c_int],
    "ipx_read_doubles": [_P, _c.c_int, _P, _P],
    "ipx_read_folded": [_c.c_int, _P, _P, _P],
    "ipx_fold_combine": [_c.c_int, _P, _P, _P, _P],
    "ipx_reduce_grid": [_I64],
    "ipx_dot_partials": [_I64, _P, _P, _P, _P],
    "ipx_norms_partials": [_I64, _P, _P, _P],
    "ipx_axpby": [_I64, _F64, _P, _F64, _P, _P, _P],
    "ipx_mul": [_I64, _P, _P, _P, _P],
    "ipx_fill": [_I64, _F64, _P, _P],
    "ipx_clip": [_I64, _P, _P, _P, _P, _P],
    "ipx_affine": [_I64, _F64, _P, _F64, _P, _P],
    "ipx_gather": [_I64, _P, _P, _P, _P, _P, _P],
    "ipx_scatter": [_I64, _P, _P, _P, _P],
    "ipx_scatter_add": [_I64, _P, _P, _P, _P],
    "ipx_max_scalar": [_I64, _P, _F64, _P, _P],
    "ipx_where_positive": [_I64, _P, _P, _F64, _P, _P],
    "ipx_assign_negated_where": [_I64, _P, _P, _P, _P],
    "ipx_sum_log": [_I64, _P, _P, _P, _P],
    "ipx_dense_gemv": [_I64, _I64, _P, _I64, _P, _F64, _P, _F64, _P, _P, _P, _P, _P],
    "ipx_gram_f64_mfma": [_I64, _I64, _P, _I64, _P, _P],
    "ipx_gram_splits": [_I64, _I64],
    "ipx_gram_f64_mfma_split": [_I64, _I64, _P, _I64, _P, _P, _I32, _P],
    "ipx_aat_dense": [_I64, _P, _P, _P, _P, _P],
    "ipx_chol_factor": [_I64, _P, _P, _P, _P],
    "ipx_chol_inverse": [_I64, _P, _P, _P],
    "ipx_trtri_lower": [_I64, _P, _P],
    "ipx_qr_factor": [_I64, _I64, _P, _I64, _P, _P, _P, _P, _P, _P, _P],
    "ipx_qr_form_q": [_I64, _I64, _P, _P, _P, _P, _P],
    "ipx_qr_wy": [_I64, _I64, _P, _P, _P, _P, _P],
    "ipx_qr_tri_inverse": [_I64, _P, _P, _P],
    "ipx_qrp_factor": [_I64, _I64, _P, _I64, _P, _P, _P, _P, _P],
    "ipx_qrp_reflectors": [_I64, _I64, _I64, _P, _P, _P, _P, _P, _P],
    "ipx_qrp_write_t": [_I64, _I64, _I64, _P, _P, _P, _P, _I64, _P],
    "ipx_qrp_fold_columns": [_I64, _I64, _I64, _P, _P, _P, _P],
    "ipx_dense_gemvt": [_I64, _I64, _P, _I64, _P, _P, _P],
    "ipx_dense_gather_rows": [_I64, _I64, _P, _I64, _P, _P, _P, _P, _I64, _I64, _P],
    "ipx_csr_rows_to_dense": [_I64, _I64, _P, _P, _P, _P, _P, _P, _P, _I64, _P],
    "ipx_dense_augment": [_I64, _I64, _I64, _P, _I64, _P, _I64, _P, _P, _P, _P],
    "ipx_gram_shift": [_I64, _I64, _P, _P, _I64, _P, _P],
    "ipx_dot": [_I64, _P, _P, _P, _P, _P],
    "ipx_norms": [_I64, _P, _P, _P, _P],
    "ipx_box_inside": [_I64, _P, _P, _P, _P, _P, _P],
    "ipx_box_sphere_reduce": [_I64, _P, _P, _F64, _P, _P, _P, _P, _P],
    "ipx_csr_tiles_host": [_I64, _P, _I32, _I32, _P, _I64],
    "ipx_csr_spmv": [_I64, _I64, _P, _P, _P, _P, _I32, _P, _F64, _P, _F64, _P, _P,
                     _c.c_int, _P, _P, _P],
    "ipx_csr_spmv_ex": [_I64, _I64, _P, _P, _P, _P, _I32, _P, _F64, _P, _F64, _P, _P, _P, _P, _P, _P],
    "ipx_fold2": [_P, _I32, _P, _P, _P],
    "ipx_cg_step1": [_I64, _P, _I32, _P, _I32, _P, _P, _P, _P, _P, _P, _P, _I32, _P],
    "ipx_cg_step2": [_I64, _P, _I32, _I32, _P, _I32, _P, _I32, _P, _I32, _P, _P, _P, _I32, _P],
    "ipx_cg_state_size": [],
    "ipx_cg_vec_grid": [_I64],
    "ipx_cg_hp": [_P, _P],
    "ipx_cg_resume": [_P, _I32, _I32, _P],
    "ipx_cg_guard_resume": [_P, _I32, _P],
    "ipx_cg_prime_state_guard": [_P, _P, _P, _F64, _F64, _F64, _F64, _F64, _P, _P],
    "ipx_cg_iterate": [_P, _I32, _I32, _P],
    "ipx_cg_resident_ok": [_P],
    "ipx_cg_prime_state": [_P, _P, _P, _F64, _F64, _F64, _F64, _F64, _P],
    "ipx_cg_prime": [_P, _P, _I32, _P, _P, _P, _P, _F64, _F64, _F64, _F64, _F64, _I32, _I32, _P],
    "ipx_cg_iterate_timed": [_P, _I32, _I32, _P, _P],
    "ipx_banded_kmax": [],
    "ipx_banded_levels": [_P],
    "ipx_banded_decoupled": [_P],
    "ipx_banded_pcr_level": [_P],
    "ipx_banded_refine_steps": [_P, _P],
    "ipx_banded_chunk_rows": [_P],
    "ipx_banded_set_decoupling": [_P, _c.c_int],
    "ipx_banded_factor": [_P, _P, _P],
    "ipx_banded_status": [_P, _P],
    "ipx_banded_solve": [_P, _P, _P, _P],
    "ipx_banded_solve_multilaunch": [_P, _P, _P, _P],
    "ipx_banded_solve_guarded_c": [_P, _P, _P, _P, _P],
    "ipx_banded_solve_resid": [_P, _P, _P, _P, _P, _P, _P],
    "ipx_banded_decoupled_geometry": [_P, _P],
    "ipx_cg_step2_hp": [_P, _I32, _I32, _P],
    "ipx_pcg_state_size": [],
    "ipx_pcg_iterate": [_P, _I32, _I32, _P],
    "ipx_pcg_coarse_max": [],
    "ipx_pcg_coarse_grid": [_I64],
    "ipx_pcg_precond_apply": [_P, _P, _P, _P, _P],
    "ipx_csr_aggregate_rows": [_I64, _P, _P, _P, _P, _P, _P, _P, _P, _P],
    "ipx_aggregate_greedy": [_I64, _P, _P, _I32, _P],
    "ipx_blockjacobi_build": [_I64, _P, _P, _P, _P, _P, _P, _P],
    "ipx_blockjacobi_apply": [_I64, _I64, _P, _P, _P, _P, _P, _P, _P],
    "ipx_cg_shard2_segment": [_P, _P, _I32, _I32, _I32, _P],
    "ipx_cg_shard2_fold_hp": [_P, _P, _P],
    "ipx_cg_shard2_iterate": [_P, _P, _I32, _I32, _P],
    "ipx_cg_shard2_fusable": [_P, _P],
    "ipx_cg_shard2_resident_ok": [_P, _P],
    "ipx_cg_shard2_resident": [_P, _P, _I32, _I32, _P],
    "ipx_cg_save_pb": [_P, _P],
    "ipx_peer_pingpong": [_P, _I32, _I32, _P, _P],
    "ipx_peer_attach_resident": [_P, _I64],
    "ipx_peer_export_resident": [_P, _P],
    "ipx_peer_import_resident": [_P, _I32, _P],
    "ipx_peer_resident_ready": [_P],
    "ipx_cg_resident_max_global": [],
    "ipx_peer_set_timeout": [_P, _F64],
    "ipx_peer_handle_bytes": [],
    "ipx_peer_export": [_P, _P],
    "ipx_peer_import": [_P, _I32, _P],
    "ipx_peer_ready": [_P],
    "ipx_peer_sequence": [_P, _P],
    "ipx_peer_allreduce": [_P, _I32, _P, _P, _P, _I32, _P],
    "ipx_peer_allgather": [_P, _I32, _P, _P, _P, _P],
    "ipx_peer_exchange": [_P, _P, _I32, _P, _P, _P],
    "ipx_aat_band": [_I64, _I32, _P, _P, _P, _P, _P, _P],
    "ipx_aat_band_w": [_I64, _I32, _P, _P, _P, _P, _P, _P, _P],
    "ipx_pairs_factor": [_I32, _P, _P, _P, _P, _P, _P, _P, _P, _P, _P, _P, _P, _P],
    "ipx_pairs_tsolve": [_I32, _P, _P, _P, _P, _P, _P, _P, _P, _P],
    "ipx_pairs_vsolve": [_I32, _P, _P, _P, _P, _P, _P, _P, _P, _P],
    "ipx_boxschur_solve": [_P, _P, _P, _P, _P, _P, _P],
    "ipx_boxschur_project": [_P, _P, _P, _P, _P, _P, _P, _P, _P],
    "ipx_boxschur_project_count": [_P],
    "ipx_banded_status_deferred": [_P, _P, _P],
    "ipx_banded_refactor": [_P, _I64, _I32, _P, _P, _P, _P, _P, _P, _P],
    "ipx_sqp_block_size": [],
    "ipx_sqp_front": [_P, _c.c_int, _c.c_int, _c.c_int, _F64, _F64, _F64, _F64, _F64, _F64, _F64,
                      _F64, _I32, _P],
    "ipx_sqp_model": [_P, _F64, _F64, _F64, _c.c_int, _P],
    "ipx_sqp_judge": [_P, _P, _F64, _P, _P],
    "ipx_sqp_refresh": [_P, _P],
    "ipx_sqp_cg_timing": [_c.c_int, _P, _P],
    "ipx_lowrank_grid": [_I64],
    "ipx_lowrank_update": [_I32, _I64, _I32, _F64, _F64, _P, _P, _P, _P, _P, _P],
    "ipx_lowrank_apply": [_I64, _I32, _P, _P, _P, _P, _I32, _P, _P],
    "ipx_csr_tdiff_dot": [_I64, _I64, _I64, _P, _P, _P, _P, _I32, _P, _P, _P, _P, _P, _P, _I32, _P],
    "ipx_csr_tdiff_dot_host": [_I64, _I64, _I64, _P, _P, _P, _P, _P, _P, _P, _P, _P, _I32],
    "ipx_fd_steps": [_I64, _I32, _F64, _P, _P, _P, _P, _P, _P, _P],
    "ipx_fd_perturb": [_I64, _I32, _I32, _P, _P, _P, _P, _P, _P, _P, _P],
    "ipx_fd_assemble": [_I64, _I64, _P, _P, _P, _I32, _I32, _P, _I32, _I32, _P, _P, _P, _P, _P,
                        _P, _P],
    "ipx_blocktri_kmax": [],
    "ipx_blocktri_levels": [_I64, _I32, _P],
    "ipx_aat_blocktri": [_I64, _I32, _I32, _P, _P, _P, _P, _P, _P, _P],
    "ipx_blocktri_factor": [_I64, _I32, _P, _P, _P, _P, _P],
    "ipx_blocktri_solve": [_I64, _I32, _P, _P, _P, _P],
    "ipx_blockwide_kmax": [],
    "ipx_blockwide_levels": [_I64, _I32, _P],
    "ipx_aat_blockwide": [_I64, _I32, _I32, _P, _P, _P, _P, _P, _P, _P],
    "ipx_blockwide_factor": [_I64, _I32, _P, _P, _P, _P, _P],
    "ipx_blockwide_solve": [_I64, _I32, _P, _P, _P, _P],
    "ipx_border_pmax": [],
# ... 19 lines not shown
_RESTYPES = {"ipx_version": _c.c_char_p, "ipx_last_error": _c.c_char_p,
             "ipx_launch_count": _c.c_longlong, "ipx_read_count": _c.c_longlong,
             "ipx_banded_create": _P, "ipx_banded_destroy": None,
             "ipx_dense_padded": _I64, "ipx_gram_ws_doubles": _I64, "ipx_peer_create": _P, "ipx_peer_destroy": None,
             "ipx_peer_halo_capacity": _I64, "ipx_peer_fused_launches": _I64,
             "ipx_cg_resident_ll_words": _I64, "ipx_cg_prime_ws_doubles": _I64,
             "ipx_peer_resident_launches": _I64, "ipx_cg_resident_limits": None,
             "ipx_sqp_part_doubles": _I64, "ipx_sqp_model_host": None, "ipx_sqp_ratio_host": None,
             "ipx_sqp_radius_host": None, "ipx_sqp_box_sphere_host": None,
             "ipx_lowrank_state_doubles": _I64, "ipx_lowrank_part_doubles": _I64,
             "ipx_lowrank_middle_host": None, "ipx_fd_steps_host": None,
             "ipx_fd_perturb_host": None, "ipx_fd_assemble_host": None,
             "ipx_fd_assemble_sym_host": None, "ipx_blocktri_ws_doubles": _I64,
             "ipx_blockwide_ws_doubles": _I64, "ipx_nd_symbolic": _I64,
             "ipx_qr_padded_cols": _I64, "ipx_qr_ws_doubles": _I64,
             "ipx_qrp_ws_doubles": _I64, "ipx_qrp_info_doubles": _I64,
             "ipx_qrp_info_ints": _I64,
             "ipx_rguard_start": _F64, "ipx_rguard_step_x": _F64, "ipx_rguard_step_q": _F64}
_EXTRA_ARGTYPES = {"ipx_blocktri_ws_doubles": [_I64, _I32],
                   "ipx_rguard_start": [_F64], "ipx_rguard_step_x": [_F64, _F64, _F64],
                   "ipx_rguard_step_q": [_F64, _F64, _F64],
                   "ipx_qr_padded_cols": [_I64], "ipx_qr_ws_doubles": [_I64, _I64],
                   "ipx_qrp_ws_doubles": [_I64, _I64], "ipx_qrp_info_doubles": [_I64],
                   "ipx_qrp_info_ints": [_I64],
                   "ipx_nd_symbolic": [_I64, _P, _P, _I32, _P, _P, _P, _P, _P, _P, _P, _I64],
                   "ipx_blockwide_ws_doubles": [_I64, _I32],
                   "ipx_banded_create": [_I64, _I32, _I32], "ipx_banded_destroy": [_P],
                   "ipx_dense_padded": [_I64], "ipx_gram_ws_doubles": [_I64, _I32],
                   "ipx_peer_create": [_I32, _I32, _I64],
                   "ipx_peer_destroy": [_P], "ipx_peer_halo_capacity": [_P],
                   "ipx_peer_fused_launches": [_P], "ipx_cg_resident_ll_words": [_I32, _I32],
                   "ipx_cg_prime_ws_doubles": [_P, _I32], "ipx_peer_resident_launches": [_P],
                   "ipx_cg_resident_limits": [_P], "ipx_sqp_part_doubles": [_P],
                   "ipx_sqp_model_host": [_P], "ipx_sqp_ratio_host": [_P],
                   "ipx_sqp_radius_host": [_P], "ipx_sqp_box_sphere_host": [_P, _F64, _c.c_int, _P],
                   "ipx_lowrank_state_doubles": [_I32], "ipx_lowrank_part_doubles": [_I64, _I32],
                   "ipx_lowrank_middle_host": [_I32, _I32, _F64, _F64, _P, _P],
                   "ipx_fd_steps_host": [_I64, _I32, _F64, _P, _P, _P, _P, _P, _P],
                   "ipx_fd_perturb_host": [_I64, _I32, _I32, _P, _P, _P, _P, _P, _P, _P],
                   "ipx_fd_assemble_host": [_I64, _I64, _P, _P, _I32, _P, _I32, _I32, _P, _P, _P,
                                            _P, _P, _P],
                   "ipx_fd_assemble_sym_host": [_I64, _P, _P, _I32, _P, _I32, _I32, _P, _P, _P, _P,
                                                _P, _P, _I32, _P]}

_lib = None


class IpxError(RuntimeError):
    pass


_ERRORS = {-1: "invalid argument", -2: "HIP launch/runtime error",
           -3: "matrix is not positive definite", -4: "out of memory",
           -5: "no path in this solver for the matrix at hand",
           -6: "factorization complete but numerically rank deficient"}


def load():
    global _lib
    if _lib is not None:
        return _lib
    if not os.path.exists(LIB_PATH):
        raise IpxError(
            "libipx.so not found at %s: build it with "
            "`python -c 'import __graft_entry__ as g; g.build()'` or "
            "`make -C ip-nonlinear-solver_amd/csrc`. This package has no CPU "
            "fallback." % LIB_PATH)
    import torch
    lib = ctypes.CDLL(LIB_PATH)
    for name, args in _SIGNATURES.items():
        fn = getattr(lib, name)
        fn.argtypes = args
        fn.restype = _c.c_int
    for name, res in _RESTYPES.items():
        getattr(lib, name).restype = res
    for name, args in _EXTRA_ARGTYPES.items():
        getattr(lib, name).argtypes = args
    _lib = lib
    return lib


DEBUG_FORMS = ("no-fuse", "no-resident", "no-compact-groups", "no-affine-groups", "keep-xn2",
               "read-xn2", "pack-comm", "no-post-tail", "no-step-chain", "no-lowrank-loop",
               "no-fused-projection", "table-columns", "no-radius-guard")


def debug_form(name):
    assert name in DEBUG_FORMS, name
    val = os.environ.get("IPX_DEBUG_FORMS", "")
    if not val:
        return False
    toks = [t.strip() for t in val.split(",") if t.strip()]
    for t in toks:
        if t not in DEBUG_FORMS:
            raise IpxError("IPX_DEBUG_FORMS: unknown form %r (known: %s)" % (t, ", ".join(DEBUG_FORMS)))
    return name in toks


def exported_symbols():
    return sorted(list(_SIGNATURES) + list(_RESTYPES))


def check(code, what=""):
    if code < 0:
        detail = load().ipx_last_error().decode() if code == -2 else ""
        raise IpxError("%s failed: %s (code %d) %s" % (what or "ipx call",
                                                       _ERRORS.get(code, "?"), code, detail))
    return code


_BOUND = {}


def call(name, *args):
    fn = _BOUND.get(name)
    if fn is None:
        fn = _BOUND[name] = getattr(load(), name)
    rc = fn(*args)
    return rc if rc >= 0 else check(rc, name)
```

ip-nonlinear-solver_amd/ipsolver/cg_fused.py:

```python
import ctypes
import os

import numpy as np
import torch

from . import _hip
from . import device as dv
from .device import DVec, DeviceCSR, _p, stream_ptr, ctx

_TINY = 1e-25
_P = ctypes.c_void_p
_I64 = ctypes.c_int64

ST_RTG0, ST_RTG1, ST_TOL, ST_RADIUS, ST_ALPHA, ST_STOP, ST_NITER, ST_BETA = range(8)
ST_PTHP, ST_ORTH_RHS, ST_XNORM2, ST_VIOL, ST_ORTH, ST_IT_DONE, ST_MARGIN = 8, 9, 10, 11, 12, 13, 14
ST_PRIME_STEPS = 15


class CgArgs(ctypes.Structure):
    _fields_ = [(name, typ) for name, typ in (
        ("n", _I64), ("m", _I64),
        ("A_rowptr", _P), ("A_colidx", _P), ("A_val", _P), ("A_tiles", _P), ("A_ntiles", _I64),
        ("At_rowptr", _P), ("At_colidx", _P), ("At_val", _P), ("At_tiles", _P), ("At_ntiles", _I64),
        ("H_rowptr", _P), ("H_colidx", _P), ("H_val", _P), ("H_tiles", _P), ("H_ntiles", _I64),
        ("H_diag", _P), ("banded", _P),
        ("x", _P), ("p", _P), ("r", _P), ("Hp", _P),
        ("w", _P), ("v", _P), ("t", _P),
        ("lb", _P), ("ub", _P), ("state", _P),
        ("part1", _P), ("part2", _P), ("part3", _P), ("part4", _P),
        ("vec_grid", _I64), ("solver_kind", _I64), ("pb", _P), ("H_hmax", _I64), ("H_tile_rows", _I64),
        ("r_next", _P), ("A_own", _P), ("A_span", _I64), ("fold_ws", _P),
        ("At_vown", _P), ("At_qv", _I64), ("A_tile_nnz", _I64),
        ("At_ell_row", _P), ("At_ell_val", _P),
        ("H_col16", _P), ("H_rowlen", _P), ("A_col16", _P), ("no_radius", _I64),
        ("A_off16", _P), ("A_rowfirst", _P), ("A_rl", _I64), ("P_win", _P), ("P_nspan", _I64),
        ("P_navn", _I64), ("H_operator", _I64),
        ("resident", _I64), ("R_ll", _P), ("R_hw", _I64), ("R_seq", _P),
        ("LR_W", _P), ("LR_state", _P), ("LR_part", _P), ("LR_mem", _I64), ("LR_rows", _I64),
        ("xsums", _P),
        ("fused_proj", _I64), ("A_ell_val", _P), ("A_ell_off16", _P), ("r_where", _P),
        ("xsums_carry", ctypes.c_int32), ("A_contig", ctypes.c_int32),
        ("rguard", _P), ("radius_guard", ctypes.c_int32))]


STATS = {"calls": 0, "iterations": 0, "batches": 0, "box_events": 0, "refine_events": 0,
         "primed_on_device": 0,
         "prime_retries": 0,
         "host_primed_directly": 0,
         "resident_calls": 0,
         "resident_fallbacks": 0,
         "operator_calls": 0,
         "radius_undecided": 0,
         "guard_lost": 0}


def _hessian_parts(H):
    from .operators import DeviceHessian
    if isinstance(H, DeviceCSR) and H.shape[0] == H.shape[1]:
        return H, None
    if isinstance(H, DeviceHessian) and H.csr is not None and not H.others \
            and H.lowrank is None:
        return H.csr, H.diag
    return None


def _lowrank_part(H):
    from .operators import DeviceHessian
    if not isinstance(H, DeviceHessian) or H.lowrank is None or H.others \
            or _hip.debug_form("no-lowrank-loop"):
        return None
    return H.lowrank


def _loop_parts(H):
    parts = _hessian_parts(H)
    if parts is not None:
        return parts[0], parts[1], None
    lr = _lowrank_part(H)
    if lr is not None:
        return H.csr, H.diag, lr
    return None


def _dense_hessian(H):
# ... 244 lines not shown
    if cache is None or cache[0] != rl:
        m = pat.shape[0]
        assert pat.nnz == m * rl
        rows = pat.indices_h.astype(np.int64).reshape(m, rl)
        off = rows - rows.min(axis=1)[:, None]
        assert off.min() >= 0 and off.max() < 65536
        src = (np.arange(m, dtype=np.int64)[None, :] * rl
               + np.arange(rl, dtype=np.int64)[:, None]).ravel()
        assert src.size == 0 or (src.min() >= 0 and src.max() < pat.nnz)
        dev = ctx().device
        contig = bool(np.array_equal(off, np.broadcast_to(np.arange(rl, dtype=np.int64), off.shape)))
        cache = pat._ipx_ellt = (
            rl, torch.from_numpy(np.ascontiguousarray(off.T).ravel().astype(np.uint16)
                                 .view(np.int16)).to(dev),
            torch.from_numpy(src.astype(np.int32)).to(dev), contig)
    _, off16, src, _ = cache
    val = torch.empty(src.numel(), dtype=torch.float64, device=off16.device)
    _hip.call("ipx_gather", src.numel(), _p(A.val), _p(src), None, None, _p(val), stream_ptr())
    A._ipx_ellt_done = (rl, off16, val)
    return off16, val


def ell_contiguous(A, rl):
    cache = getattr(A.pattern, "_ipx_ellt", None)
    return cache is not None and cache[0] == rl and cache[3]


def _solver_kind(solver):
    from .projector import BandedNormalSolver
    from .boxschur import BoxSchurNormalSolver
    if isinstance(solver, BandedNormalSolver):
        return 0 if solver.perm is None else None
    if isinstance(solver, BoxSchurNormalSolver):
        return 1 if solver.c_args() is not None else None
    return None


def supports(H, Z, Y):
    from .projector import NormalEquationProjector
    P = getattr(Z, "projector", None)
    if P is None or getattr(Y, "projector", None) is not P:
        return False
    if not isinstance(P, NormalEquationProjector):
        return False
    from .dense import DeviceDense, DenseNormalSolver
    if isinstance(P.A, DeviceDense):
        return (P.m > 0 and isinstance(P.solver, DenseNormalSolver)
                and not getattr(P.solver, "refine_steps", 0)
                and (_dense_hessian(H) is not None or _loop_parts(H) is not None))
    if not isinstance(P.A, DeviceCSR):
        return False
    if P.m == 0 or _solver_kind(P.solver) is None:
        return False
    return _loop_parts(H) is not None or hasattr(H, "dot")


def _ptr(t):
    return ctypes.c_void_p(t.data_ptr()) if t is not None else None


_POOL = {}
POOL_STATS = {"built": 0, "reused": 0}


def _signature(H, P, lb, ub):
    from .dense import DeviceDense
    if isinstance(P.A, DeviceDense):
        return None
    parts = _loop_parts(H)
    if parts is None:
        return None
    Hc, Hd, LR = parts
    flags = os.environ.get("IPX_DEBUG_FORMS", "")
    return (id(Hc.pattern) if Hc is not None else None, Hd is None, id(P.A.pattern), lb is None,
            ub is None, _solver_kind(P.solver), int(getattr(P.solver, "k", 0)), flags,
            id(LR.mem) if LR is not None else None)


def _loop_for(H, P, lb, ub):
    key = _signature(H, P, lb, ub)
    L = _POOL.pop(key, None) if key is not None else None
    if L is not None and L.rebind(H, P, lb, ub):
        POOL_STATS["reused"] += 1
        L.enqueued = None
        if key in _NO_RESIDENT:
            L.args.resident = 0
        return L, key
    POOL_STATS["built"] += 1
    L = _Loop(H, P, lb, ub, resident=False if key in _NO_RESIDENT else None, arm=False)
    L.enqueued = None
    return L, key


def _release(L, key):
    L.args.radius_guard = 0
    if key is None:
        return
    if len(_POOL) >= 4:
        _POOL.pop(next(iter(_POOL)))
    _POOL[key] = L


class _Loop:

    def rebind(self, H, P, lb, ub):
        lib = _hip.load()
        a = self.args
        A = P.A
        At = A.T
        Hc, Hd, LR = _loop_parts(H)
        if a.solver_kind == 0:
            geo = (ctypes.c_int32 * 2)()
            ok = bool(lib.ipx_banded_decoupled_geometry(ctypes.c_void_p(P.solver.handle), geo))
            if (ok, geo[0], geo[1]) != self.geometry:
                return False
            if self.pcr_L is not None and \
                    int(lib.ipx_banded_pcr_level(ctypes.c_void_p(P.solver.handle))) != self.pcr_L:
                if getattr(self, "proj_tabs", None) is not None:
                    return False
                self.fp_tabs, self.pcr_L = None, None
            a.banded = ctypes.c_void_p(P.solver.handle)
        else:
            a.banded = ctypes.cast(ctypes.pointer(P.solver.c_args()), ctypes.c_void_p)
        a.A_val, a.At_val = _ptr(A.val), _ptr(At.val)
        a.H_val = _ptr(Hc.val) if Hc is not None else None
        a.H_diag = _ptr(Hd.t) if Hd is not None else None
        self.lowrank = LR
        self._bind_lowrank(LR)
        a.lb = _ptr(lb.t) if lb is not None else None
        a.ub = _ptr(ub.t) if ub is not None else None
        if a.At_ell_val:
            self.ell_row, self.ell_val = ell_rows(At, self.row_rel)
            a.At_ell_row, a.At_ell_val = _ptr(self.ell_row), _ptr(self.ell_val)
        a.fused_proj = 0
        a.no_radius = 0
        a.xsums_carry = 0
        a.radius_guard = 0
        if self.xsums is not None:
            self.xsums.zero_()
        if self.rguard is not None:
            self.rguard.zero_()
        self.x = torch.empty(self.n, dtype=torch.float64, device=self.state.device)
        a.x = _ptr(self.x)
        self.keep = (A, At, Hc, Hd, lb, ub, P, LR)
        return True

    def arm_fused_projection(self, iterations=None):
        if getattr(self, "fp_tabs", None) is None:
            return False
        a, A = self.args, self.keep[0]
        done = getattr(A, "_ipx_ellt_done", None)
        current = done is not None and done[0] == self.fp_tabs[2]
        if not current and iterations is not None and iterations < FUSED_MIN_BATCH:
            a.fused_proj = 0
            return False
        self.A_ell_off16, self.A_ell_val = ell_transposed(A, self.fp_tabs[2])
        a.A_ell_off16, a.A_ell_val = _ptr(self.A_ell_off16), _ptr(self.A_ell_val)
        a.A_contig = 1 if ell_contiguous(A, self.fp_tabs[2]) \
            and not _hip.debug_form("table-columns") else 0
        a.fused_proj = 1
        return True

    def arm_radius_guard(self, key, trust_radius, has_box):
        a = self.args
        a.radius_guard = 0
        if self.rguard is None or self.xsums is None or has_box or a.no_radius \
                or not np.isfinite(trust_radius) or a.resident \
                or _hip.debug_form("no-radius-guard") or (key is not None and key in _GUARD_LOST):
            return False
        a.radius_guard = 1
        return True

    def _bind_lowrank(self, LR):
        a = self.args
        if LR is None:
            a.LR_W = a.LR_state = a.LR_part = None
            a.LR_mem = a.LR_rows = 0
            return
        m = LR.mem
        a.LR_W, a.LR_state, a.LR_part = _ptr(m.W), _ptr(m.state), _ptr(m.part)
        a.LR_mem, a.LR_rows = m.strategy.memory, m.n

    def _part1_doubles(self, count):
        lr = self.lowrank
        if lr is not None:
            count = max(count, _hip.load().ipx_lowrank_grid(lr.mem.n))
        return 2 * max(count, 1)

    def __init__(self, H, P, lb, ub, resident=None, fused_projection=None, arm=True):
        from .dense import DeviceDense
        self.geometry, self.pcr_L, self.operator = None, None, None
        self.xsums = None
        self.rguard = None
        self.fp_tabs = None
        if isinstance(P.A, DeviceDense):
            self._init_dense(H, P, lb, ub)
            return
        lib = _hip.load()
        A = P.A
        At = A.T
        parts = _loop_parts(H)
        self.operator = None if parts is not None else H
        Hc, Hd, LR = parts if parts is not None else (None, None, None)
        self.lowrank = LR
        self.n, self.m = P.n, P.m
        n, m = self.n, self.m
        dev = ctx().device
        f64 = torch.float64
        self.x = torch.empty(n, dtype=f64, device=dev)
        self.p = torch.empty(n, dtype=f64, device=dev)
        self.r = torch.empty(n, dtype=f64, device=dev)
        self.Hp = torch.empty(n, dtype=f64, device=dev)
        self.w = torch.empty(m, dtype=f64, device=dev)
        self.v = torch.empty(m, dtype=f64, device=dev)
        self.t = torch.empty(m, dtype=f64, device=dev)
        self.state = torch.zeros(lib.ipx_cg_state_size(), dtype=f64, device=dev)
        grid = lib.ipx_cg_vec_grid(n)
        self.part1 = torch.zeros(self._part1_doubles(Hc.pattern.ntiles if Hc is not None else 1),
                                 dtype=f64, device=dev)
        self.part2 = torch.zeros(2 * max(grid, A.pattern.ntiles, n // 1024 + 2), dtype=f64,
                                 device=dev)
        self.part3 = torch.zeros(2 * max(At.pattern.ntiles, (m + 255) // 256 + 1, n // 1024 + 2),
                                 dtype=f64, device=dev)
        self.part4 = torch.zeros((m + 255) // 256 + 1, dtype=f64, device=dev)
        self.keep = (A, At, Hc, Hd, lb, ub, P, LR)
        a = CgArgs()
        self.args = a
        a.n, a.m = n, m
# ... 212 lines not shown
                    STATS["prime_retries"] += 1
            if key is not None:
                if len(_HOST_PRIMED) >= 16:
                    _HOST_PRIMED.clear()
                _HOST_PRIMED.add(key)
    steps = None
    if key is not None and key in _HOST_PRIMED:
        steps = P.stats["refinements"] + P.stats["cancellation_steps"]
        STATS["host_primed_directly"] += 1
    out = _projected_cg(H, c, Z, Y, b, trust_radius, lb, ub, tol, max_iter,
                        max_infeasible_iter, batch, stats, b_zero, fast=False)
    if steps is not None and P.stats["refinements"] + P.stats["cancellation_steps"] == steps:
        _HOST_PRIMED.discard(key)
    return out


_HOST_PRIMED = set()
_GUARD_LOST = set()
_STEP_PRIMED = set()


_PRIME_IDX = (ctypes.c_int32 * 7)(12, 4, 0, 2, 10, 6, 8)
_PRIME_IDX_B0 = (ctypes.c_int32 * 7)(-1, 4, 0, 2, 10, 6, 8)


def _prime_without_reads(L, H, c, Z, Y, b, b_zero, P, tol, trust_radius):
    n = len(c)
    ctx_ = ctx()
    if b_zero:
        x0 = DVec.zeros(n)
        t = c
    else:
        x0 = Y.dot(-b)
        _hip.call("ipx_norms", n, _p(x0.t), ctypes.c_void_p(ctx_.out.data_ptr() + 8 * 12),
                  _p(ctx_.ws), stream_ptr())
        t = H.dot(x0) + c
    r0 = P.null_space_enqueue(t, 0)
    g0 = P.null_space_enqueue(r0, 6)
    _hip.call("ipx_cg_prime_state_guard", _p(L.state), _p(ctx_.out),
              _PRIME_IDX_B0 if b_zero else _PRIME_IDX,
              float("nan") if tol is None else float(tol), float(trust_radius),
              float(P.orth_tol), float(P.norm_A), float(P.CANCELLATION),
              _p(L.rguard) if L.args.radius_guard else None, stream_ptr())
    return x0, r0, g0


def _projected_cg(H, c, Z, Y, b, trust_radius, lb, ub, tol, max_iter, max_infeasible_iter,
                  batch, stats, b_zero, fast):
    from . import qp
    lib = _hip.load()
    P = Z.projector
    n, m = len(c), len(b)
    has_box = lb is not None or ub is not None
    ub_given = ub is not None
    if has_box:
        lb = lb if lb is not None else DVec.full(n, -np.inf)
        ub = ub if ub is not None else DVec.full(n, np.inf)
    if max_iter is None:
        max_iter = n - m
    max_iter = min(max_iter, n - m)
    if max_infeasible_iter is None:
        max_infeasible_iter = n - m
    if fast:
        L, pool_key = _loop_for(H, P, lb if has_box else None,
                                ub if has_box and ub_given else None)
        if L.operator is not None:
            _release(L, pool_key)
            raise _PrimeRetry()
        if np.isinf(trust_radius) and trust_radius > 0 and not has_box \
                and not _hip.debug_form("keep-xn2"):
            L.args.no_radius = 1
        L.arm_radius_guard(pool_key, trust_radius, has_box)
        st = stream_ptr()
        a = L.args
        if isinstance(P.A, DeviceCSR) and a.solver_kind in (0, 1) and getattr(P.solver, "perm", None) is None \
                and a.banded and not getattr(P.solver, "refine_steps", 0) and L.lowrank is None \
                and lib.ipx_cg_prime_ws_doubles(L.ref(), P.A.pattern.ntiles) <= 65536:
            ctx_ = ctx()
            pat = P.A.pattern
            first_end = min(max_iter, batch if batch else _first_batch(max_iter, False))
            L.arm_fused_projection(first_end)
            b_rows = None if b_zero else P.rows_in(b)
            L.stepped = bool(b_zero and pool_key is not None and pool_key in _STEP_PRIMED)
            _hip.call("ipx_cg_prime", L.ref(), _p(pat.tiles), pat.ntiles, _p(c.t),
                      None if b_zero else _p(b_rows.t), _p(ctx_.out), _p(ctx_.ws),
                      float("nan") if tol is None else float(tol), float(trust_radius),
                      float(P.orth_tol), float(P.norm_A), float(P.CANCELLATION),
                      max(first_end, 0), 1 if L.stepped else 0, st)
            L.enqueued = (0, first_end) if first_end > 0 else None
            P.stats["solves"] += 2 if b_zero else 3
        else:
            x0, r0, g0 = _prime_without_reads(L, H, c, Z, Y, b, b_zero, P, tol, trust_radius)
            L.x.copy_(x0.t)
            L.r.copy_(r0.t)
            _hip.call("ipx_axpby", n, -1.0, _p(g0.t), 0.0, None, _p(L.p), st)
            _hip.check(lib.ipx_cg_hp(L.ref(), st), "ipx_cg_hp")
        STATS["primed_on_device"] += 1
        return _run_loop(L, pool_key, P, lib, st, n, lb, ub, trust_radius, max_iter,
                         max_infeasible_iter, batch, stats, fast=True)

    if b_zero:
        x0 = DVec.zeros(n)
        r0 = Z.dot(c)
        norm_x0 = 0.0
    else:
        x0 = Y.dot(-b)
        r0 = Z.dot(H.dot(x0) + c)
        norm_x0 = None
    g0 = Z.dot(r0)
    red = getattr(P, "_red", None)
    rt_g = float(red[0]) if red is not None and P.m > 0 else g0.sumsq_amax()[0]
    tr_distance = trust_radius - (dv.norm(x0) if norm_x0 is None else norm_x0)
    if tr_distance < 0:
        raise ValueError("Trust region problem does not have a solution.")
    if tr_distance < _TINY:
        return x0, {'niter': 0, 'stop_cond': 2, 'hits_boundary': True}

    if tol is None:
        tol = max(min(0.01 * np.sqrt(rt_g), 0.1 * rt_g), _TINY)

    L, pool_key = _loop_for(H, P, lb if has_box else None, ub if has_box and ub_given else None)
    if np.isinf(trust_radius) and trust_radius > 0 and not has_box \
            and not _hip.debug_form("keep-xn2"):
        L.args.no_radius = 1
    if L.arm_radius_guard(pool_key, trust_radius, has_box):
        nx0 = dv.norm(x0) if norm_x0 is None else norm_x0
        L.rguard.copy_(torch.tensor([nx0 * lib.ipx_rguard_start(1.0), lib.ipx_rguard_start(rt_g),
                                     0.0], dtype=torch.float64))
    L.arm_fused_projection(min(max_iter, batch if batch
                                else _first_batch(max_iter, L.operator is not None)))
    st = stream_ptr()
    L.x.copy_(x0.t)
    L.r.copy_(r0.t)
    _hip.call("ipx_axpby", n, -1.0, _p(g0.t), 0.0, None, _p(L.p), st)
    init = np.zeros(L.state.numel())
    init[ST_RTG0] = rt_g
    init[ST_TOL] = tol
    init[ST_RADIUS] = trust_radius
    init[ST_ORTH_RHS] = P.orth_tol * P.norm_A
    L.state.copy_(torch.from_numpy(init))
    _hip.check(lib.ipx_cg_hp(L.ref(), st), "ipx_cg_hp")
    if L.operator is not None:
        L.apply_operator()
        STATS["operator_calls"] += 1
    return _run_loop(L, pool_key, P, lib, st, n, lb, ub, trust_radius, max_iter,
                     max_infeasible_iter, batch, stats, fast=False)


def _first_batch(max_iter, operator):
    if operator:
        return 2
    return max_iter if 4 < max_iter <= 32 else 4


def _run_loop(L, pool_key, P, lib, st, n, lb, ub, trust_radius, max_iter, max_infeasible_iter,
              batch, stats, fast, primed_state=None, release=True, first_batch=None):
    pending = [primed_state]

    _fb = first_batch if first_batch else _first_batch(max_iter, L.operator is not None)

    class Driver:
        first_batch = _fb
        batch_cap = 64 if L.operator is None else 8
        carry_at = None
        settled = True

        def iterate(self, it, end):
            self.last = (it, end)
            carry, self.carry_at = self.carry_at == it, None
            if getattr(L, "enqueued", None) is not None:
                done, L.enqueued = L.enqueued, None
                if done == (it, end):
                    return
                raise _hip.IpxError("device loop: the batch enqueued with the priming %r is not "
                                    "the one the driver asks for %r" % (done, (it, end)))
            if not L.args.fused_proj and self.settled:
                L.arm_fused_projection(end - it)
            if L.operator is None:
                L.args.xsums_carry = 1 if carry else 0
                try:
                    _hip.check(lib.ipx_cg_iterate(L.ref(), it, end, st), "ipx_cg_iterate")
                finally:
                    L.args.xsums_carry = 0
            else:
                for k in range(it, end):
                    _hip.check(lib.ipx_cg_iterate(L.ref(), k, k + 1, st), "ipx_cg_iterate")
                    L.apply_operator()

        def read_state(self):
            mine = pending[0] is None
            if not mine:
                s, pending[0] = list(pending[0]), None
            else:
                s = dv.read_doubles(L.state, L.state.numel())
            self.settled = int(s[ST_STOP]) == 0
            if mine and int(s[ST_STOP]) == 0 and not L.args.resident and L.xsums is not None:
                self.carry_at = self.last[1]
            for watch in _WATCH_BATCHES:
                watch(L, self.last)
            if fast and int(s[ST_STOP]) == 9:
                if release:
                    _release(L, pool_key)
                raise _PrimeRetry()
            if fast and pool_key is not None and getattr(L, "stepped", None) is not None:
                if s[ST_PRIME_STEPS] > 0 or s[ST_MARGIN] < 64.0 * P.CANCELLATION ** 2:
                    _STEP_PRIMED.add(pool_key)
                else:
                    _STEP_PRIMED.discard(pool_key)
                L.stepped = None
            if _INJECT_RESIDENT_TIMEOUT and L.args.resident and int(s[ST_STOP]) in (0, 4):
                _INJECT_RESIDENT_TIMEOUT.pop()
                L.x[: L.n // 2] += 1.0
                L.state[ST_STOP] = 8.0
                s = list(s)
                s[ST_STOP] = 8.0
            if int(s[ST_STOP]) == 8 and L.args.resident:
                STATS["resident_fallbacks"] += 1
                if pool_key is not None:
                    _NO_RESIDENT.add(pool_key)
                L.args.resident = 0
                L.state[ST_STOP] = 0.0
                raise _ResidentGaveUp()
            return s

        def X(self):
            return DVec(L.x)

        def Pv(self):
            return DVec(L.p)

        def set_x(self, v):
            L.x = v.t

        def zeros(self):
            return DVec.zeros(n)

        def resume(self, it_stop, mode):
            self.carry_at = None
            return _resume(lib, L, it_stop, mode, st)

        def refine(self, it_stop):
            self.carry_at = None
            _refine(P, L, DVec(L.g_tensor(it_stop)))

        guard_lost = False

        def guard_resume(self, it_stop):
            self.guard_lost = True
            L.args.radius_guard = 0
            L.state[ST_STOP] = 0.0
            _hip.check(lib.ipx_cg_guard_resume(L.ref(), it_stop, st), "ipx_cg_guard_resume")
            s = dv.read_doubles(L.state, L.state.numel())
            self.settled = int(s[ST_STOP]) == 0
            self.carry_at = it_stop + 1 if self.settled else None
            return s

    D = Driver()
    x, niter, stop_cond, hits_boundary = run_device_loop(
        D, STATS, lb, ub, trust_radius, max_iter, max_infeasible_iter, batch, stats)
    if pool_key is not None:
        if D.guard_lost:
            if len(_GUARD_LOST) >= 16:
                _GUARD_LOST.clear()
            _GUARD_LOST.add(pool_key)
        elif not hits_boundary:
            _GUARD_LOST.discard(pool_key)
    STATS["calls"] += 1
    STATS["iterations"] += niter
    STATS["resident_calls"] += 1 if L.args.resident else 0
    if release:
        _release(L, pool_key)
    return x, {'niter': niter, 'stop_cond': stop_cond, 'hits_boundary': hits_boundary}


def run_device_loop(D, counters, lb, ub, trust_radius, max_iter, max_infeasible_iter,
                    batch=None, stats=None):
    from . import qp
    has_box = lb is not None or ub is not None
    hits_boundary, stop_cond = False, 1
    counter, last_viol_it = 0, -2
    last_feasible_x = D.zeros() if has_box else None
    it = 0
    nbatch = batch if batch else D.first_batch
    s = None
    while it < max_iter:
        end = min(max_iter, it + nbatch)
        D.iterate(it, end)
        s = D.read_state()
        counters["batches"] += 1
        if stats is not None:
            stats["batches"] = stats.get("batches", 0) + 1
        stop = int(s[ST_STOP])
        if stop == 0:
            it = end
            if not batch:
                nbatch = min(2 * nbatch, D.batch_cap)
            continue
        it_stop = int(s[ST_IT_DONE])
        if stop == 11:
            counters["guard_lost"] = counters.get("guard_lost", 0) + 1
            s = D.guard_resume(it_stop)
            stop = int(s[ST_STOP])
            if stop == 0:
                it = it_stop + 1
                continue
        alpha = s[ST_ALPHA]
        if stop == 4:
            stop_cond = 4
            break
        if stop == 3:
            if np.isinf(trust_radius):
                raise ValueError("Negative curvature not allowed "
                                 "for unrestrited problems.")
            X, Pv = D.X(), D.Pv()
            _, al, hit = qp.box_sphere_intersections(X, Pv, lb, ub, trust_radius,
                                                     entire_line=True)
            xf = X.add_scaled(Pv, al) if hit else X
            D.set_x(qp.reinforce_box_boundaries(xf, lb, ub))
            stop_cond, hits_boundary = 3, True
            break
        undecided = stop == 10
        if undecided:
            counters["radius_undecided"] = counters.get("radius_undecided", 0) + 1
            if dv.norm(D.X().add_scaled(D.Pv(), alpha)) >= trust_radius:
                stop = 2
        if stop == 2:
            X, Pv = D.X(), D.Pv()
            _, theta, hit = qp.box_sphere_intersections(X, Pv, lb, ub, trust_radius,
                                                        dscale=alpha)
            xf = X.add_scaled(Pv, theta * alpha) if hit else X
            D.set_x(qp.reinforce_box_boundaries(xf, lb, ub))
            stop_cond, hits_boundary = 2, True
            break
        mode = 0
        if stop == 5:
            counters["box_events"] += 1
            if last_viol_it != it_stop - 1:
                counter = 0
            counter += 1
            last_viol_it = it_stop
            X, Pv = D.X(), D.Pv()
            _, theta, hit = qp.box_sphere_intersections(X, Pv, lb, ub, trust_radius,
                                                        dscale=alpha)
            if hit:
                last_feasible_x = qp.reinforce_box_boundaries(
                    X.add_scaled(Pv, theta * alpha), lb, ub)
                counter = 0
                last_viol_it = -2
            if counter > max_infeasible_iter:
                break
        if stop == 5 or undecided:
            mode = 1
            s = D.resume(it_stop, mode)
            if int(s[ST_STOP]) == 6:
                stop, mode = 6, 1
            else:
                it = it_stop + 1
                continue
        if stop == 6:
            counters["refine_events"] += 1
            D.refine(it_stop)
            s = D.resume(it_stop, mode | 3)
            it = it_stop + 1
            continue
        if stop == 7:
            raise _hip.IpxError("sharded projected CG: a wait on the peer mailboxes timed out "
                                "(a rank of the group died or fell out of step; iteration %d, "
                                "wait code %s)" % (it_stop, s[ST_VIOL]))
        raise _hip.IpxError("unexpected CG stop code %d" % stop)

    x = D.X()
    if has_box and not qp.inside_box_boundaries(x, lb, ub):
        x = last_feasible_x
        hits_boundary = True
# ... 30 lines not shown
```

Before: 31580 iterations/s.

## Move CG batch loop into C with published state reads and fused priming tails

The Python batch driver loop, which iterated, read state and doubled the batch size, now runs inside a C entry point (ipx_cg_run). Each batch's state is published to a host-visible buffer with a tagged store, folded into the residual settle kernel. Priming also fuses the Y(-b) solve with the A^T product through a new no-residual PCR kernel variant. Zeroing of xsums/rguard and saving of the p boundaries are folded into the prime-state kernel, and the Python-side zero_ calls are deferred. The aim is fewer launches and less Python/ctypes overhead per batch, at the cost of added complexity and new tag-based host–device synchronisation paths.

```diff
diff --git a/include/ipx.h b/include/ipx.h
--- a/include/ipx.h
+++ b/include/ipx.h
@@ -245,6 +245,15 @@
 int ipx_cg_prime_state(double *state, const double *red, const int32_t *idx7, double tol_in,
                        double radius, double orth_tol, double norm_A, double cancellation,
                        void *stream);
+int ipx_cg_batch_plan(int32_t max_iter, int32_t first, int32_t cap, int32_t fixed, int32_t *out,
+                      int32_t n_out);
+int ipx_cg_run(const ipx_cg_args *a, int32_t it, int32_t max_iter, int32_t first_batch,
+               int32_t batch_cap, int32_t fixed_batch, int32_t carry, uint32_t pending_tag,
+               double *state_out, int32_t *batches_out, int32_t *last_out, void *stream);
+int ipx_cg_prime_pub(const ipx_cg_args *a, const int32_t *A_tiles, int32_t A_ntiles,
+                     const double *c, const double *b, double *red, double *ws, double tol_in,
+                     double radius, double orth_tol, double norm_A, double cancellation,
+                     int32_t first_end, int32_t steps, uint32_t *tag_out, void *stream);
 int ipx_cg_iterate_timed(const ipx_cg_args *a, int32_t it_begin, int32_t it_end,
                          float *ms_out, void *stream);
 int ipx_cg_step1(int64_t n, double *state, int32_t it, const double *p1, int32_t np1,
diff --git a/ip-nonlinear-solver_amd/csrc/banded.hip b/ip-nonlinear-solver_amd/csrc/banded.hip
--- a/ip-nonlinear-solver_amd/csrc/banded.hip
+++ b/ip-nonlinear-solver_amd/csrc/banded.hip
@@ -1273,7 +1273,7 @@
   }
 }
 
-template <int QV, int NR, bool ROWS, int TB, bool POST = false>
+template <int QV, int NR, bool ROWS, int TB, bool POST = false, bool NOR = false>
 __global__ void __launch_bounds__(TB)
 k_solve_pcr(int m, int rows_wg, int L, int nwin, const double *__restrict__ band,
             const double *__restrict__ w, double *__restrict__ x, double *__restrict__ partial,
@@ -1350,7 +1350,8 @@
   v2d ar[QP];
   if (QV > 0)
     tail.load(atv.ell_row, atv.ell_val, atv.ell_n, av0, avn, tid, [&](int k, int64_t j) {
-      ar[k] = *reinterpret_cast<const v2d *>(atv.r_in + j);
+      if constexpr (NOR) ar[k] = (v2d){0.0, 0.0};
+      else ar[k] = *reinterpret_cast<const v2d *>(atv.r_in + j);
     });
   int pg0 = 0, pgn = 0, pe0 = 0, pen = 0;
   int py0[POST ? POST_PG + 1 : 1], py1[POST ? POST_PG + 1 : 1];
@@ -1489,6 +1490,20 @@
   return IPX_OK;
 }
 
+template <int QV>
+int launch_solve_pcr_nor_q(const LevDev &lv, int L, const double *w, double *x, int *npartial,
+                           const AtvJob &atv, hipStream_t st) {
+  const int rows_wg = DEC_CHUNKS * lv.q;
+  const int grid = (lv.P + DEC_CHUNKS - 1) / DEC_CHUNKS;
+  if (rows_wg + 2 * (1 << L) > PCR_TB) return IPX_EUNSUPPORTED;
+  if (npartial) *npartial = grid;
+  hipLaunchKernelGGL((k_solve_pcr<QV, 1, false, PCR_TB, false, true>), dim3(ipx_xcd_grid(grid)),
+                     dim3(PCR_TB), 0, st, lv.m, rows_wg, L, grid, lv.band, w, x, nullptr, nullptr,
+                     atv, RowsJob{});
+  IPX_CHECK_LAUNCH();
+  return IPX_OK;
+}
+
 int launch_solve_pcr_rows(const LevDev &lv, int L, const RowsJob &rows, double *x,
                           double *partial, int *npartial, const double *guard, hipStream_t st,
                           const PostJob *post = nullptr) {
@@ -2562,6 +2577,29 @@
                            &job, qv);
 }
 
+int ipx_banded_solve_atv_only_launch(void *handle, const double *w, double *x, double *g_out,
+                                     const int32_t *vown, int qv, double *part3, int *npartial,
+                                     const uint16_t *ell_row, const double *ell_val,
+                                     int64_t ell_n, double sign, hipStream_t st) {
+  if (!handle || !w || !x || !g_out || !vown || !part3 || w == x ||
+      (sign != 1.0 && sign != -1.0))
+    return IPX_EINVAL;
+  int32_t geo[2];
+  if (!ipx_banded_decoupled_geometry(handle, geo)) return IPX_EUNSUPPORTED;
+  Banded *h = (Banded *)handle;
+  if (h->pcr_L <= 0 || h->lev[0].k != 1 || !ell_row || !ell_val || qv <= 0 || (ell_n & 1))
+    return IPX_EUNSUPPORTED;
+  const AtvJob job{nullptr, nullptr, nullptr, nullptr, g_out, vown, part3, ell_row, ell_val, ell_n,
+                   sign};
+  const LevDev lv = to_dev(h->lev[0], nullptr);
+  const int per = pcr_tail_per_lane(qv);
+  if (per <= 2) return launch_solve_pcr_nor_q<2>(lv, h->pcr_L, w, x, npartial, job, st);
+  if (per <= 4) return launch_solve_pcr_nor_q<4>(lv, h->pcr_L, w, x, npartial, job, st);
+  if (per <= 6) return launch_solve_pcr_nor_q<6>(lv, h->pcr_L, w, x, npartial, job, st);
+  if (per <= 8) return launch_solve_pcr_nor_q<8>(lv, h->pcr_L, w, x, npartial, job, st);
+  return IPX_EUNSUPPORTED;
+}
+
 int ipx_banded_fused_proj_ok(void *handle, int rl, int64_t nspan, int qv) {
   int32_t geo[2];
   if (!handle || !ipx_banded_decoupled_geometry(handle, geo)) return IPX_EUNSUPPORTED;
diff --git a/ip-nonlinear-solver_amd/csrc/cg.hip b/ip-nonlinear-solver_amd/csrc/cg.hip
--- a/ip-nonlinear-solver_amd/csrc/cg.hip
+++ b/ip-nonlinear-solver_amd/csrc/cg.hip
@@ -876,6 +876,25 @@
     dst[i] = src[i];
 }
 
+struct CgPub { unsigned int *dst; unsigned int tag; };
+typedef unsigned int cg_u4 __attribute__((ext_vector_type(4)));
+__global__ void __launch_bounds__(VB)
+k_cg_settle_publish(int64_t n, const int32_t *__restrict__ where, const double *__restrict__ src,
+                    double *__restrict__ dst, const double *__restrict__ state, CgPub pub) {
+  if (blockIdx.x == 0 && threadIdx.x < ST_SIZE) {
+    const unsigned long long bits =
+        (unsigned long long)__double_as_longlong(state[threadIdx.x]);
+    cg_u4 w;
+    w.x = (unsigned)(bits & 0xffffffffull); w.y = pub.tag;
+    w.z = (unsigned)(bits >> 32);           w.w = pub.tag;
+    cg_u4 *d = (cg_u4 *)pub.dst + threadIdx.x;
+    asm volatile("global_store_dwordx4 %0, %1, off sc0 sc1" ::"v"(d), "v"(w) : "memory");
+  }
+  if (!where || *where == 0) return;
+  for (int64_t i = (int64_t)blockIdx.x * VB + threadIdx.x; i < n; i += (int64_t)gridDim.x * VB)
+    dst[i] = src[i];
+}
+
 __global__ void k_xsums_void(double *xs_tag) { *xs_tag = 0.0; }
 
 __global__ void k_rguard_advance(const double *__restrict__ st, int parity, double *rg) {
@@ -1232,7 +1251,8 @@
                                a->p, a->Hp, a->H_diag, has_base ? 1 : 0, a->part1, guard, st);
 }
 
-int launch_hp(const ipx_cg_args *a, const LoopPlan &P, const double *guard, hipStream_t st) {
+int launch_hp(const ipx_cg_args *a, const LoopPlan &P, const double *guard, hipStream_t st,
+              bool boundaries_saved = false) {
   int rc = IPX_OK;
   switch (P.hp) {
     case HP_OPERATOR:
@@ -1253,7 +1273,7 @@
     }
   }
   if (!rc && P.lowrank_tail) rc = launch_lowrank(a, true, guard, st);
-  if (rc || P.hp != HP_CSR || !P.fused_hp) return rc;
+  if (rc || P.hp != HP_CSR || !P.fused_hp || boundaries_saved) return rc;
   return launch_save_pb(a, st);
 }
 
@@ -1477,10 +1497,11 @@
 #undef MARK
 
 int cg_iterate(const ipx_cg_args *a, const LoopPlan &P, int32_t it_begin, int32_t it_end,
-               hipStream_t st, hipEvent_t *ev) {
+               hipStream_t st, hipEvent_t *ev, const CgPub *pub = nullptr) {
   if (P.proj == PJ_DENSE) {
     if (ev) return IPX_EINVAL;
   } else if (!ev && it_end > it_begin && ipx_cg_resident_ok(a)) {
+    if (pub) return IPX_EINVAL;
     int rc = ipx_cg_resident_launch(a, it_begin, it_end, P.np1, P.np2, P.np3, P.np4, st);
     if (rc || !P.fused_hp) return rc;
     return launch_save_pb(a, st);
@@ -1508,6 +1529,14 @@
     if (rc) return rc;
     rc = launch_update_half(a, P, h, a->part2, np2, a->part3, np3, a->part4, np4, st);
     if (rc) return rc;
+  }
+  if (pub) {
+    const bool settle = P.proj == PJ_STEP1_SOLVE_TAIL && it_end > it_begin;
+    hipLaunchKernelGGL(k_cg_settle_publish, dim3(settle ? ipx_grid_for(a->n, VB * 4, 1024) : 1),
+                       dim3(VB), 0, st, a->n, settle ? (const int32_t *)a->r_where : nullptr,
+                       (const double *)a->r_next, a->r, (const double *)a->state, *pub);
+    IPX_CHECK_LAUNCH();
+    return IPX_OK;
   }
   if (P.proj == PJ_STEP1_SOLVE_TAIL && it_end > it_begin) {
     hipLaunchKernelGGL(k_cg_settle_r, dim3(ipx_grid_for(a->n, VB * 4, 1024)), dim3(VB), 0, st, a->n,
@@ -1866,12 +1895,31 @@
   red[PR_TAKEN + pj] = 0.0;
 }
 
+struct PrimeTail {
+  const double *p;
+  const int32_t *tiles;
+  double *pb, *zero, *rguard_zero;
+  int ntiles, hmax, nzero;
+};
 __global__ void __launch_bounds__(IPX_BLOCK)
 k_cg_prime_state_folds(double *st, double *red, PrimeFolds f, ipx_prime_idx ix, double tol_in,
                        double radius, double orth_tol, double norm_A, double canc2,
                        const double *__restrict__ radius_dev,
                        const double *__restrict__ norm_A2_dev, PrimeStep last, int have_last,
-                       double *rguard) {
+                       double *rguard, PrimeTail tail) {
+  if (blockIdx.x > 0) {
+    const int idx = ((int)blockIdx.x - 1) * IPX_BLOCK + (int)threadIdx.x;
+    if (idx < tail.nzero) tail.zero[idx] = 0.0;
+    if (idx < 3 && tail.rguard_zero) tail.rguard_zero[idx] = 0.0;
+    if (idx < tail.ntiles * 2 * tail.hmax) {
+      const int t = idx / (2 * tail.hmax), j = idx - t * 2 * tail.hmax;
+      const int r0 = tail.tiles[t], r1 = tail.tiles[t + 1];
+      const double v = j < tail.hmax ? tail.p[r0 + j] : tail.p[r1 - tail.hmax + (j - tail.hmax)];
+      tail.pb[idx] = v;
+      tail.pb[(int64_t)tail.ntiles * 2 * tail.hmax + idx] = v;
+    }
+    return;
+  }
   if (radius_dev) radius = *radius_dev;
   if (norm_A2_dev) norm_A = sqrt(*norm_A2_dev);
   __shared__ double lds[12 * (IPX_BLOCK / IPX_WAVE)];
@@ -2062,7 +2110,87 @@
                  int32_t steps, void *stream) {
   return ipx_cg_prime_dev(a, A_tiles, A_ntiles, c, b, red, ws, tol_in, radius, nullptr, orth_tol,
                           norm_A, nullptr, cancellation, first_end, steps, nullptr, 0, 0,
-                          (hipStream_t)stream);
+                          (hipStream_t)stream, nullptr, 0);
+}
+
+}
+
+static int cg_run_batches(const ipx_cg_args *a0, int64_t it, int64_t max_iter, int64_t nbatch,
+                          int64_t cap, bool fixed, int carry, bool pending, CgPub pub,
+                          double *state_out, int32_t *batches_out, int32_t *last_out,
+                          hipStream_t st) {
+  ipx_cg_args a = *a0;
+  const LoopPlan P = plan_of(&a);
+  int nb = 0, rc = IPX_OK;
+  while (true) {
+    const int64_t end = std::min(max_iter, it + nbatch);
+    if (!pending) {
+      rc = ipx_read_begin(&pub.dst, &pub.tag);
+      if (rc) break;
+      a.xsums_carry = carry;
+      rc = cg_iterate(&a, P, (int32_t)it, (int32_t)end, st, nullptr, &pub);
+      if (rc) break;
+    }
+    pending = false;
+    rc = ipx_read_wait(pub.dst, pub.tag, ST_SIZE, state_out, st);
+    if (rc) break;
+    ++nb;
+    if (last_out) { last_out[0] = (int32_t)it; last_out[1] = (int32_t)end; last_out[2] = (int32_t)nbatch; }
+    if (state_out[ST_STOP] != 0.0 || end >= max_iter) break;
+    it = end;
+    carry = 1;
+    if (!fixed) nbatch = std::min(2 * nbatch, cap);
+  }
+  if (batches_out) *batches_out = nb;
+  return rc;
+}
+
+extern "C" {
+
+int ipx_cg_batch_plan(int32_t max_iter, int32_t first, int32_t cap, int32_t fixed, int32_t *out,
+                      int32_t n_out) {
+  if (max_iter < 0 || cap < 1 || fixed < 0 || (fixed == 0 && first < 1) || (n_out > 0 && !out))
+    return IPX_EINVAL;
+  int64_t it = 0, nbatch = fixed > 0 ? fixed : first;
+  int nb = 0;
+  while (it < max_iter) {
+    it = std::min<int64_t>(max_iter, it + nbatch);
+    if (nb < n_out) out[nb] = (int32_t)it;
+    ++nb;
+    if (fixed == 0) nbatch = std::min<int64_t>(2 * nbatch, cap);
+  }
+  return nb;
+}
+
+int ipx_cg_run(const ipx_cg_args *a, int32_t it, int32_t max_iter, int32_t first_batch,
+               int32_t batch_cap, int32_t fixed_batch, int32_t carry, uint32_t pending_tag,
+               double *state_out, int32_t *batches_out, int32_t *last_out, void *stream) {
+  if (!a || !state_out || it < 0 || it >= max_iter || batch_cap < 1 || fixed_batch < 0 ||
+      (fixed_batch == 0 && first_batch < 1) || a->H_operator || ipx_cg_resident_ok(a))
+    return IPX_EINVAL;
+  CgPub pub{nullptr, pending_tag};
+  if (pending_tag != 0) {
+    const int rc = ipx_read_buffer(&pub.dst);
+    if (rc) return rc;
+  }
+  return cg_run_batches(a, it, max_iter, fixed_batch > 0 ? fixed_batch : first_batch, batch_cap,
+                        fixed_batch > 0, carry != 0 ? 1 : 0, pending_tag != 0, pub, state_out,
+                        batches_out, last_out, (hipStream_t)stream);
+}
+
+int ipx_cg_prime_pub(const ipx_cg_args *a, const int32_t *A_tiles, int32_t A_ntiles,
+                     const double *c, const double *b, double *red, double *ws, double tol_in,
+                     double radius, double orth_tol, double norm_A, double cancellation,
+                     int32_t first_end, int32_t steps, uint32_t *tag_out, void *stream) {
+  if (!a || !tag_out || first_end < 1 || ipx_cg_resident_ok(a)) return IPX_EINVAL;
+  CgPub pub{nullptr, 0};
+  int rc = ipx_read_begin(&pub.dst, &pub.tag);
+  if (rc) return rc;
+  rc = ipx_cg_prime_dev(a, A_tiles, A_ntiles, c, b, red, ws, tol_in, radius, nullptr, orth_tol,
+                        norm_A, nullptr, cancellation, first_end, steps, nullptr, 0, 0,
+                        (hipStream_t)stream, pub.dst, pub.tag);
+  *tag_out = rc ? 0 : pub.tag;
+  return rc;
 }
 
 }
@@ -2072,7 +2200,7 @@
                      double radius, const double *radius_dev, double orth_tol, double norm_A,
                      const double *norm_A2_dev, double cancellation, int32_t first_end,
                      int steps, const double *c_part, int32_t c_npart, int x_is_zero,
-                     hipStream_t stream) {
+                     hipStream_t stream, unsigned int *pub_dst, unsigned int pub_tag) {
   if (!a || !c || !red || !ws || !A_tiles || a->solver_kind > 1 || a->m <= 0 || a->H_operator ||
       !a->H_rowptr || !a->t || first_end < 0 || a->LR_W)
     return IPX_EINVAL;
@@ -2088,9 +2216,26 @@
   int rc;
   const double *t = c;
   if (b) {
-    rc = prime_solve(a, b, a->v, stream);
-    if (rc) return rc;
-    rc = R.spmv(At, a->v, -1.0, nullptr, 0.0, nullptr, a->x, 12, st);
+    rc = IPX_EUNSUPPORTED;
+    const int cap = (int)((a->m + 255) / 256) + 8;
+    if ((P.proj == PJ_SOLVE_TAIL || P.proj == PJ_STEP1_SOLVE_TAIL) && a->At_ell_row &&
+        a->At_ell_val &&
+        8 * (int64_t)cap + 2 * a->H_ntiles + 4096 <= IPX_WS_DOUBLES) {
+      int np = 0;
+      rc = ipx_banded_solve_atv_only_launch(a->banded, b, a->v, a->x, a->At_vown, (int)a->At_qv,
+                                            R.ws + R.off, &np, a->At_ell_row, a->At_ell_val,
+                                            a->n, 1.0, st);
+      if (rc == IPX_OK) {
+        if (np > cap) return IPX_EINVAL;
+        R.single(R.ws + R.off, np, 12);
+        R.off += 2 * (int64_t)cap;
+      }
+    }
+    if (rc == IPX_EUNSUPPORTED) {
+      rc = prime_solve(a, b, a->v, stream);
+      if (rc) return rc;
+      rc = R.spmv(At, a->v, -1.0, nullptr, 0.0, nullptr, a->x, 12, st);
+    }
     if (rc) return rc;
     rc = R.spmv(Hm, a->x, 1.0, a->H_diag, 1.0, c, a->Hp, 4, st);
     if (rc) return rc;
@@ -2122,13 +2267,25 @@
   const int32_t idx_b[7] = {12, 4, 0, 2, 0, 6, 8}, idx_0[7] = {-1, 4, 0, 2, 0, 6, 8};
   ipx_prime_idx ix;
   for (int k = 0; k < 7; ++k) ix.i[k] = (b ? idx_b : idx_0)[k];
-  hipLaunchKernelGGL(k_cg_prime_state_folds, dim3(1), dim3(IPX_BLOCK), 0, st, a->state, red, R.f,
-                     ix, tol_in, radius, orth_tol, norm_A, canc2, radius_dev, norm_A2_dev, s2,
-                     (b || !steps) ? 0 : 1, a->radius_guard != 0 ? a->rguard : nullptr);
+  const bool guard_on = a->radius_guard != 0 && a->rguard != nullptr;
+  PrimeTail tail{};
+  if (P.hp == HP_CSR && P.fused_hp) {
+    tail.p = a->p; tail.tiles = a->H_tiles; tail.pb = a->pb;
+    tail.ntiles = (int)a->H_ntiles; tail.hmax = (int)a->H_hmax;
+  }
+  if (a->xsums) { tail.zero = a->xsums; tail.nzero = 3 * (int)a->H_ntiles + 770; }
+  if (!guard_on) tail.rguard_zero = a->rguard;
+  const int tail_n = std::max(std::max(tail.ntiles * 2 * tail.hmax, tail.nzero),
+                              tail.rguard_zero ? 3 : 0);
+  hipLaunchKernelGGL(k_cg_prime_state_folds, dim3(1 + (tail_n + IPX_BLOCK - 1) / IPX_BLOCK),
+                     dim3(IPX_BLOCK), 0, st, a->state, red, R.f, ix, tol_in, radius, orth_tol,
+                     norm_A, canc2, radius_dev, norm_A2_dev, s2, (b || !steps) ? 0 : 1,
+                     guard_on ? a->rguard : nullptr, tail);
   IPX_CHECK_LAUNCH();
-  rc = launch_hp(a, P, nullptr, st);
+  rc = launch_hp(a, P, nullptr, st, true);
   if (rc || first_end == 0) return rc;
-  return cg_iterate(a, P, 0, first_end, st, nullptr);
+  const CgPub pub{pub_dst, pub_tag};
+  return cg_iterate(a, P, 0, first_end, st, nullptr, pub_dst ? &pub : nullptr);
 }
 
 extern "C" {
diff --git a/ip-nonlinear-solver_amd/csrc/ipx_common.h b/ip-nonlinear-solver_amd/csrc/ipx_common.h
--- a/ip-nonlinear-solver_amd/csrc/ipx_common.h
+++ b/ip-nonlinear-solver_amd/csrc/ipx_common.h
@@ -10,6 +10,7 @@
 
 void ipx_note_error(hipError_t e, const char *file, int line);
 int ipx_read_begin(unsigned int **pinned_out, unsigned int *tag_out);
+int ipx_read_buffer(unsigned int **pinned_out);
 int ipx_read_wait(unsigned int *pinned, unsigned int tag, int k, double *host_out, hipStream_t st);
 int ipx_read_ints(const int *dev, int k, int *host_out, hipStream_t st);
 
@@ -512,7 +513,8 @@
                      double radius, const double *radius_dev, double orth_tol, double norm_A,
                      const double *norm_A2_dev, double cancellation, int32_t first_end,
                      int steps, const double *c_part, int32_t c_npart, int x_is_zero,
-                     hipStream_t stream);
+                     hipStream_t stream, unsigned int *pub_dst = nullptr,
+                     unsigned int pub_tag = 0);
 
 struct ipx_csr_view {
   int nrows, ncols;
@@ -562,6 +564,10 @@
                                       double sign = 1.0);
 int ipx_banded_solve_resid_launch(void *handle, const double *w, double *x, double *partial,
                                   int *npartial, const double *guard, hipStream_t st);
+int ipx_banded_solve_atv_only_launch(void *handle, const double *w, double *x, double *g_out,
+                                     const int32_t *vown, int qv, double *part3, int *npartial,
+                                     const uint16_t *ell_row, const double *ell_val,
+                                     int64_t ell_n, double sign, hipStream_t st);
 constexpr int IPX_XS_SLICE = 64;
 constexpr int IPX_XS_STRIDE = IPX_BLOCK;
 constexpr int IPX_RG_X = 0, IPX_RG_Q = 1, IPX_RG_T = 2;
diff --git a/ip-nonlinear-solver_amd/csrc/misc.hip b/ip-nonlinear-solver_amd/csrc/misc.hip
--- a/ip-nonlinear-solver_amd/csrc/misc.hip
+++ b/ip-nonlinear-solver_amd/csrc/misc.hip
@@ -26,9 +26,8 @@
   snprintf(g_last_error, sizeof(g_last_error), "%s (%s:%d)", hipGetErrorString(e), file, line);
 }
 
-int ipx_read_begin(unsigned int **pinned_out, unsigned int *tag_out) {
+int ipx_read_buffer(unsigned int **pinned_out) {
   static thread_local unsigned int *pinned = nullptr;
-  static thread_local unsigned int seq = 0;
   if (!pinned) {
     if (hipHostMalloc((void **)&pinned, IPX_READ_MAX * 16, hipHostMallocMapped | hipHostMallocCoherent) != hipSuccess) {
       pinned = nullptr;
@@ -36,8 +35,15 @@
     }
     memset(pinned, 0, IPX_READ_MAX * 16);
   }
+  *pinned_out = pinned;
+  return IPX_OK;
+}
+
+int ipx_read_begin(unsigned int **pinned_out, unsigned int *tag_out) {
+  static thread_local unsigned int seq = 0;
+  const int rc = ipx_read_buffer(pinned_out);
+  if (rc != IPX_OK) return rc;
   if (++seq == 0) ++seq;
-  *pinned_out = pinned;
   *tag_out = seq;
   return IPX_OK;
 }
diff --git a/ip-nonlinear-solver_amd/ipsolver/_hip.py b/ip-nonlinear-solver_amd/ipsolver/_hip.py
--- a/ip-nonlinear-solver_amd/ipsolver/_hip.py
+++ b/ip-nonlinear-solver_amd/ipsolver/_hip.py
@@ -74,6 +74,10 @@
     "ipx_cg_prime_state": [_P, _P, _P, _F64, _F64, _F64, _F64, _F64, _P],
     "ipx_cg_prime": [_P, _P, _I32, _P, _P, _P, _P, _F64, _F64, _F64, _F64, _F64, _I32, _I32, _P],
     "ipx_cg_iterate_timed": [_P, _I32, _I32, _P, _P],
+    "ipx_cg_batch_plan": [_I32, _I32, _I32, _I32, _P, _I32],
+    "ipx_cg_run": [_P, _I32, _I32, _I32, _I32, _I32, _I32, _c.c_uint32, _P, _P, _P, _P],
+    "ipx_cg_prime_pub": [_P, _P, _I32, _P, _P, _P, _P, _F64, _F64, _F64, _F64, _F64, _I32, _I32,
+                         _P, _P],
     "ipx_banded_kmax": [],
     "ipx_banded_levels": [_P],
     "ipx_banded_decoupled": [_P],
@@ -259,7 +263,7 @@
 
 DEBUG_FORMS = ("no-fuse", "no-resident", "no-compact-groups", "no-affine-groups", "keep-xn2",
                "read-xn2", "pack-comm", "no-post-tail", "no-step-chain", "no-lowrank-loop",
-               "no-fused-projection", "table-columns", "no-radius-guard")
+               "no-fused-projection", "table-columns", "no-radius-guard", "python-batch-loop")
 
 
 def debug_form(name):
diff --git a/ip-nonlinear-solver_amd/ipsolver/cg_fused.py b/ip-nonlinear-solver_amd/ipsolver/cg_fused.py
--- a/ip-nonlinear-solver_amd/ipsolver/cg_fused.py
+++ b/ip-nonlinear-solver_amd/ipsolver/cg_fused.py
@@ -1,5 +1,6 @@
 import ctypes
 import os
+import threading
 
 import numpy as np
 import torch
@@ -410,13 +411,14 @@
     L = _POOL.pop(key, None) if key is not None else None
     if L is not None and L.rebind(H, P, lb, ub):
         POOL_STATS["reused"] += 1
-        L.enqueued = None
+        L.enqueued, L.pending_tag = None, 0
         if key in _NO_RESIDENT:
             L.args.resident = 0
         return L, key
     POOL_STATS["built"] += 1
     L = _Loop(H, P, lb, ub, resident=False if key in _NO_RESIDENT else None, arm=False)
     L.enqueued = None
+    L.pending_tag = 0
     return L, key
 
 
@@ -464,14 +466,19 @@
         a.no_radius = 0
         a.xsums_carry = 0
         a.radius_guard = 0
-        if self.xsums is not None:
-            self.xsums.zero_()
-        if self.rguard is not None:
-            self.rguard.zero_()
+        self.sums_stale = True
         self.x = torch.empty(self.n, dtype=torch.float64, device=self.state.device)
         a.x = _ptr(self.x)
         self.keep = (A, At, Hc, Hd, lb, ub, P, LR)
         return True
+
+    def clear_sums(self):
+        if getattr(self, "sums_stale", False):
+            if self.xsums is not None:
+                self.xsums.zero_()
+            if self.rguard is not None:
+                self.rguard.zero_()
+        self.sums_stale = False
 
     def arm_fused_projection(self, iterations=None):
         if getattr(self, "fp_tabs", None) is None:
@@ -850,14 +857,24 @@
             L.arm_fused_projection(first_end)
             b_rows = None if b_zero else P.rows_in(b)
             L.stepped = bool(b_zero and pool_key is not None and pool_key in _STEP_PRIMED)
-            _hip.call("ipx_cg_prime", L.ref(), _p(pat.tiles), pat.ntiles, _p(c.t),
-                      None if b_zero else _p(b_rows.t), _p(ctx_.out), _p(ctx_.ws),
-                      float("nan") if tol is None else float(tol), float(trust_radius),
-                      float(P.orth_tol), float(P.norm_A), float(P.CANCELLATION),
-                      max(first_end, 0), 1 if L.stepped else 0, st)
+            prime_args = (L.ref(), _p(pat.tiles), pat.ntiles, _p(c.t),
+                          None if b_zero else _p(b_rows.t), _p(ctx_.out), _p(ctx_.ws),
+                          float("nan") if tol is None else float(tol), float(trust_radius),
+                          float(P.orth_tol), float(P.norm_A), float(P.CANCELLATION))
+            L.pending_tag = 0
+            if first_end > 0 and _batches_in_c(L):
+                o = _run_out()
+                _hip.call("ipx_cg_prime_pub", *prime_args, first_end, 1 if L.stepped else 0,
+                          o.tag_p, st)
+                L.pending_tag = int(o.tag.value)
+            else:
+                _hip.call("ipx_cg_prime", *prime_args, max(first_end, 0), 1 if L.stepped else 0,
+                          st)
             L.enqueued = (0, first_end) if first_end > 0 else None
+            L.sums_stale = False
             P.stats["solves"] += 2 if b_zero else 3
         else:
+            L.clear_sums()
             x0, r0, g0 = _prime_without_reads(L, H, c, Z, Y, b, b_zero, P, tol, trust_radius)
             L.x.copy_(x0.t)
             L.r.copy_(r0.t)
@@ -888,6 +905,7 @@
         tol = max(min(0.01 * np.sqrt(rt_g), 0.1 * rt_g), _TINY)
 
     L, pool_key = _loop_for(H, P, lb if has_box else None, ub if has_box and ub_given else None)
+    L.clear_sums()
     if np.isinf(trust_radius) and trust_radius > 0 and not has_box \
             and not _hip.debug_form("keep-xn2"):
         L.args.no_radius = 1
@@ -921,6 +939,40 @@
     return max_iter if 4 < max_iter <= 32 else 4
 
 
+_BATCH_CAP = 64
+
+
+def _batches_in_c(L):
+    a = L.args
+    return L.operator is None and a.solver_kind == 0 and not a.resident and not a.lb \
+        and not a.ub and not _WATCH_BATCHES and not _INJECT_RESIDENT_TIMEOUT \
+        and not _hip.debug_form("python-batch-loop")
+
+
+def _arming_settled(L):
+    return bool(L.args.fused_proj) or getattr(L, "fp_tabs", None) is None
+
+
+class _RunOut(threading.local):
+
+    def __init__(self):
+        self.state = (ctypes.c_double * 16)()
+        self.nb = ctypes.c_int32(0)
+        self.last = (ctypes.c_int32 * 3)()
+        self.tag = ctypes.c_uint32(0)
+        self.state_p = ctypes.addressof(self.state)
+        self.nb_p = ctypes.addressof(self.nb)
+        self.last_p = ctypes.addressof(self.last)
+        self.tag_p = ctypes.addressof(self.tag)
+
+
+_RUN_OUT = _RunOut()
+
+
+def _run_out():
+    return _RUN_OUT
+
+
 def _run_loop(L, pool_key, P, lib, st, n, lb, ub, trust_radius, max_iter, max_infeasible_iter,
               batch, stats, fast, primed_state=None, release=True, first_batch=None):
     pending = [primed_state]
@@ -929,7 +981,7 @@
 
     class Driver:
         first_batch = _fb
-        batch_cap = 64 if L.operator is None else 8
+        batch_cap = _BATCH_CAP if L.operator is None else 8
         carry_at = None
         settled = True
 
@@ -955,12 +1007,36 @@
                     _hip.check(lib.ipx_cg_iterate(L.ref(), k, k + 1, st), "ipx_cg_iterate")
                     L.apply_operator()
 
+        def run_batches(self, it, nbatch, max_iter, fixed):
+            if primed_state is not None or not _batches_in_c(L):
+                return None
+            end = min(max_iter, it + nbatch)
+            tag = 0
+            if getattr(L, "enqueued", None) is not None:
+                tag = getattr(L, "pending_tag", 0)
+                if not tag or L.enqueued != (it, end):
+                    return None
+                L.enqueued, L.pending_tag = None, 0
+            elif not L.args.fused_proj and self.settled:
+                L.arm_fused_projection(end - it)
+            carry, self.carry_at = self.carry_at == it, None
+            o = _run_out()
+            _hip.call("ipx_cg_run", L.ref(), it, max_iter if _arming_settled(L) else end,
+                      nbatch, self.batch_cap, nbatch if fixed else 0, 1 if carry else 0, tag,
+                      o.state_p, o.nb_p, o.last_p, st)
+            nb, last = int(o.nb.value), tuple(o.last)
+            self.last = (last[0], last[1])
+            return self._look_at(list(o.state), True), nb, last[0], last[1], last[2]
+
         def read_state(self):
             mine = pending[0] is None
             if not mine:
                 s, pending[0] = list(pending[0]), None
             else:
                 s = dv.read_doubles(L.state, L.state.numel())
+            return self._look_at(s, mine)
+
+        def _look_at(self, s, mine):
             self.settled = int(s[ST_STOP]) == 0
             if mine and int(s[ST_STOP]) == 0 and not L.args.resident and L.xsums is not None:
                 self.carry_at = self.last[1]
@@ -1051,13 +1127,18 @@
     it = 0
     nbatch = batch if batch else D.first_batch
     s = None
+    run_batches = getattr(D, "run_batches", None)
     while it < max_iter:
         end = min(max_iter, it + nbatch)
-        D.iterate(it, end)
-        s = D.read_state()
-        counters["batches"] += 1
+        ahead = run_batches(it, nbatch, max_iter, bool(batch)) if run_batches else None
+        if ahead is not None:
+            s, nb, it, end, nbatch = ahead
+        else:
+            D.iterate(it, end)
+            s, nb = D.read_state(), 1
+        counters["batches"] += nb
         if stats is not None:
-            stats["batches"] = stats.get("batches", 0) + 1
+            stats["batches"] = stats.get("batches", 0) + nb
         stop = int(s[ST_STOP])
         if stop == 0:
             it = end
```

Measured after the change: 31760 iterations/s (median of 6 runs). No clear change (+0.6%).
